# barlettacarmen/CrCNN

Measured on NVIDIA B200. Metric: encrypted MNIST images/sec, higher is better.
Workload: dtype u64

## Files before the change

### crcnn_b200/csrc/engine.cu

```cuda
#include <cuda_runtime.h>
#include <dlfcn.h>
#include <algorithm>
#include <cstdlib>
#include <cstring>
#include <map>
#include <unordered_map>
#include <string>
#include <vector>

#include "../../include/crcnn_b200.h"
#include "kernels.cuh"
#include "params.h"
#include "tc_mac.cuh"
#include "tcn_mac.cuh"
#include "relin32.cuh"
#include "reenc.cuh"

using namespace crcnn;

namespace {

enum KernelClass {
    KC_NTT_FWD = 0, KC_NTT_INV, KC_MAC, KC_PLAIN_EXPAND, KC_POOL, KC_BN, KC_PLAIN_OP,
    KC_BEHZ_LIFT, KC_SQ_TENSOR, KC_BEHZ_FLOOR, KC_RELIN, KC_PROBE, KC_TC_SPLIT, KC_TC_MAC, KC_TCN_SPLIT, KC_TCN_MAC, KC_RELIN32, KC_REENC, KC_COUNT
};
const char *kClassNames[KC_COUNT] = {"ntt_forward", "ntt_inverse", "weighted_sum_mac", "plain_expand_ntt", "pool_sum",
                                     "batch_norm", "plain_op", "behz_lift", "square_tensor", "behz_floor_sk",
                                     "relinearize", "imad_probe", "tc_plane_split", "weighted_sum_tc_i8", "tcn_plane_split",
                                     "weighted_sum_tcn_i8", "relinearize_u32", "reencrypt"};

thread_local std::string g_create_error;

}

struct crcnn_tensor {
    long count;
    int size;
    int ntt;
    uint64_t *d;
};

static long next_plain_serial() { static long s = 0; return ++s; }

struct crcnn_plain {
    long serial = next_plain_serial();
    long count;
    bool sparse_shape = false;
    std::vector<uint32_t> off, idx;
    std::vector<uint64_t> val;
    uint32_t *d_off = nullptr, *d_idx = nullptr;
    uint64_t *d_val = nullptr;
    uint64_t *ntt_mul = nullptr;
    uint64_t *ntt_mul_sh = nullptr;
    uint64_t *ntt_add = nullptr;
    uint64_t *coef_add = nullptr;
    int tap_state = 0;
    int tc_state = 0;
    int8_t *tc_A = nullptr;
    int tc_R = 0, tc_Kpad = 0;
    uint8_t *tcn_W = nullptr;
    int tcn_R = 0;
    uint64_t *fused_C = nullptr, *fused_Csh = nullptr, *fused_D = nullptr;
    long fused_scale = 0, fused_mean = 0;
    int add_mult = 1;
    bool dense_only = false;
    crcnn_plain *folded_w = nullptr, *folded_b = nullptr;
    long folded_key[9] = {0, 0, 0, 0, 0, 0, 0, 0, 0};
};

struct crcnn_evk {
    uint64_t *d = nullptr;
    long key_off[MAXK];
    int digits[MAXK];
    int dbc;
    bool has_r32 = false;
    Relin32 r32;
};

struct crcnn_keys {
    uint64_t *sk = nullptr;
    uint64_t *pk = nullptr;
    ReencConsts c;
};

struct crcnn_ctx {
    int device = 0;
    cudaStream_t stream = nullptr;
    HostParams hp;
    DeviceParams *dP = nullptr;
    std::vector<void *> owned;
    int n = 0, logn = 0, K = 0, S = 0;
    int chunk_terms = 1 << 30;
    size_t weight_cache_bytes = 24ull << 30;
    int sm_count = 148;
    int tc_mode = 1;
    int tc_min_fanin = 256;
    int tc_min_outputs = 32;
    int tap_mode = 1;
    int relin_mode = 1;
    int tcn_mode = 1;
    int tcn_fold = 1;
    size_t tc_scratch_bytes = 12ull << 30;
    std::string err;
    std::map<std::vector<int>, int *> index_cache;
    std::unordered_map<void *, size_t> big_size;
    std::multimap<size_t, void *> big_free;
    size_t big_cached = 0, big_cache_cap = 64ull << 30;
    long long st_big_malloc = 0, st_big_hit = 0, st_big_bypass = 0, st_flush = 0, st_small_malloc = 0;
    uint64_t *stage = nullptr;
    size_t stage_bytes = 0;
    bool prof_on = false;
    long launches[KC_COUNT] = {0};
    double ms[KC_COUNT] = {0};
    double work_bytes[KC_COUNT] = {0};
    double work_ops[KC_COUNT] = {0};
    struct Pending { int cls; cudaEvent_t a, b; };
    std::vector<Pending> pending;
    std::vector<cudaEvent_t> event_pool;
};

namespace {

int fail(crcnn_ctx *ctx, int code, const std::string &msg) {
    if (ctx) ctx->err = msg; else g_create_error = msg;
    return code;
}

#define CU(call)                                                                                       \
    do {                                                                                               \
        cudaError_t e__ = (call);                                                                      \
        if (e__ != cudaSuccess) {                                                                      \
            int code__ = (e__ == cudaErrorMemoryAllocation) ? CRCNN_ERR_OUT_OF_MEMORY : CRCNN_ERR_CUDA; \
            return fail(ctx, code__, std::string(#call) + ": " + cudaGetErrorString(e__));            \
        }                                                                                              \
    } while (0)

#define REQUIRE(cond, msg) \
    do { if (!(cond)) return fail(ctx, CRCNN_ERR_INVALID_ARGUMENT, msg); } while (0)

struct ProfScope {
    crcnn_ctx *c; int cls; cudaEvent_t a = nullptr, b = nullptr;
    ProfScope(crcnn_ctx *ctx, int k, double bytes = 0, double ops = 0) : c(ctx), cls(k) {
        c->launches[cls]++;
        c->work_bytes[cls] += bytes;
        c->work_ops[cls] += ops;
        if (!c->prof_on) return;
        auto get = [&]() { cudaEvent_t e; if (!c->event_pool.empty()) { e = c->event_pool.back(); c->event_pool.pop_back(); } else cudaEventCreate(&e); return e; };
        a = get(); b = get();
        cudaEventRecord(a, c->stream);
    }
    ~ProfScope() {
        if (!a) return;
        cudaEventRecord(b, c->stream);
        c->pending.push_back({cls, a, b});
    }
};

void prof_collect(crcnn_ctx *c) {
    for (auto &p : c->pending) {
        cudaEventSynchronize(p.b);
        float t = 0;
        cudaEventElapsedTime(&t, p.a, p.b);
        c->ms[p.cls] += t;
        c->event_pool.push_back(p.a);
        c->event_pool.push_back(p.b);
    }
    c->pending.clear();
}

inline size_t poly_words(const crcnn_ctx *c) { return (size_t)c->K * c->n; }
inline double lp_bytes(const crcnn_ctx *c, double polys) { return polys * c->n * 8.0; }
inline double lp_bfly(const crcnn_ctx *c, double polys) { return polys * (c->n / 2) * c->logn; }

constexpr size_t kBigBlock = 32ull << 20;
void big_cache_flush(crcnn_ctx *ctx) {
    for (auto &kv : ctx->big_free) { ctx->big_size.erase(kv.second); cudaFreeAsync(kv.second, ctx->stream); }
    ctx->big_free.clear();
    ctx->big_cached = 0;
}
int dev_alloc(crcnn_ctx *ctx, size_t bytes, void **out) {
    *out = nullptr;
    if (bytes == 0) return CRCNN_OK;
    if (bytes >= kBigBlock) {
        auto it = ctx->big_free.find(bytes);
        if (it != ctx->big_free.end()) {
            *out = it->second;
            ctx->big_cached -= bytes;
            ctx->big_free.erase(it);
            ctx->st_big_hit++;
            return CRCNN_OK;
        }
        ctx->st_big_malloc++;
    } else {
        ctx->st_small_malloc++;
    }
    cudaError_t e = cudaMallocAsync(out, bytes, ctx->stream);
    if (e == cudaErrorMemoryAllocation && !ctx->big_free.empty()) {
        cudaGetLastError();
        ctx->st_flush++;
        big_cache_flush(ctx);
        e = cudaMallocAsync(out, bytes, ctx->stream);
    }
    CU(e);
    if (bytes >= kBigBlock) ctx->big_size[*out] = bytes;
    return CRCNN_OK;
}
void dev_free(crcnn_ctx *ctx, void *p) {
    if (!p) return;
    auto it = ctx->big_size.find(p);
    if (it != ctx->big_size.end()) {
        if (ctx->big_cached + it->second <= ctx->big_cache_cap) {
            ctx->big_free.insert({it->second, p});
            ctx->big_cached += it->second;
            return;
        }
        ctx->big_size.erase(it);
        ctx->st_big_bypass++;
    }
    cudaFreeAsync(p, ctx->stream);
}

int new_tensor(crcnn_ctx *ctx, long count, int size, int ntt, crcnn_tensor **out) {
    auto *t = new crcnn_tensor{count, size, ntt, nullptr};
    int rc = dev_alloc(ctx, (size_t)count * size * poly_words(ctx) * 8, (void **)&t->d);
    if (rc) { delete t; return rc; }
    *out = t;
    return CRCNN_OK;
}

int ntt_inplace(crcnn_ctx *ctx, uint64_t *d, long npolys, int slot_base, int slot_count, bool inverse) {
    ProfScope ps(ctx, inverse ? KC_NTT_INV : KC_NTT_FWD, 2 * lp_bytes(ctx, npolys), lp_bfly(ctx, npolys));
    CU(launch_ntt(ctx->dP, ctx->logn, d, npolys, slot_base, slot_count, inverse, ctx->stream));
    return CRCNN_OK;
}

int ensure_domain(crcnn_ctx *ctx, crcnn_tensor *t, int want_ntt) {
    if (t->ntt == want_ntt) return CRCNN_OK;
    int rc = ntt_inplace(ctx, t->d, t->count * t->size * ctx->K, 0, ctx->K, !want_ntt);
    if (rc) return rc;
    t->ntt = want_ntt;
    return CRCNN_OK;
}

enum PlainForm { PF_NTT_MUL, PF_NTT_ADD, PF_COEF_ADD };

int expand_range(crcnn_ctx *ctx, crcnn_plain *p, long first, long count, PlainForm f, uint64_t *dst) {
    ProfScope ps(ctx, KC_PLAIN_EXPAND, lp_bytes(ctx, (double)count * ctx->K), f != PF_COEF_ADD ? lp_bfly(ctx, (double)count * ctx->K) : 0);
    CU(launch_plain_expand(ctx->dP, ctx->logn, ctx->K, p->d_off, p->d_idx, p->d_val, first, count,
                           (f == PF_NTT_MUL ? 0 : 1) | (p->sparse_shape ? 2 : 0), f != PF_COEF_ADD, dst, ctx->stream));
    return CRCNN_OK;
}

int ensure_form(crcnn_ctx *ctx, crcnn_plain *p, PlainForm f) {
// ... 173 lines not shown
    TcnSplitArgs s{};
    s.src = w->ntt_mul; s.index = nullptr; s.dst = w->tcn_W; s.item_polys = 1;
    s.R = R; s.Kpad = Kpad; s.planes = 7; s.ncols = Mall; s.slot0 = 0; s.nslots = ctx->K * ctx->n; s.n = ctx->n; s.K = ctx->K;
    {
        ProfScope ps(ctx, KC_TCN_SPLIT, lp_bytes(ctx, (double)w->count * ctx->K) + (double)tcn_w_bytes(7, Mall, Kpad, ctx->K, ctx->n), 0);
        CU(launch_tcn_split(s, ctx->stream));
    }
    dev_free(ctx, w->ntt_mul); w->ntt_mul = nullptr;
    if (w->ntt_mul_sh) { dev_free(ctx, w->ntt_mul_sh); w->ntt_mul_sh = nullptr; }
    w->tcn_R = R;
    return CRCNN_OK;
}

int run_weighted_sum_tcn(crcnn_ctx *ctx, crcnn_tensor *in, crcnn_plain *w, crcnn_plain *b, const int *d_index, int R,
                         int Npos, int Pimg, int m_first, int M, crcnn_tensor *out) {
    int rc = ensure_domain(ctx, in, 1);
    if (!rc) rc = ensure_form(ctx, b, PF_NTT_ADD);
    if (!rc) rc = ensure_tcn_weights(ctx, w, R);
    if (rc) return rc;
    const size_t pw = poly_words(ctx);
    const int Kpad = tcn_kpad(R), ncols = 2 * Npos, total = ctx->K * ctx->n;
    const size_t per_slot = tcn_x_bytes_per_slot(7, ncols, Kpad);
    long chunk = (long)(ctx->tc_scratch_bytes / per_slot) / 32 * 32;
    chunk = std::max<long>(32, std::min<long>(chunk, total));
    uint8_t *scratch = nullptr;
    rc = dev_alloc(ctx, (size_t)chunk * per_slot, (void **)&scratch);
    if (rc) return rc;
    TcnSplitArgs s{};
    s.src = in->d; s.index = d_index; s.dst = scratch; s.item_polys = 2;
    s.R = R; s.Kpad = Kpad; s.planes = 7; s.ncols = ncols; s.n = ctx->n; s.K = ctx->K;
    TcnMacArgs a{};
    a.W = w->tcn_W; a.X = scratch; a.bias = b->ntt_add + (size_t)m_first * pw; a.out = out->d;
    a.Mall = (int)(w->count / R); a.m_first = m_first; a.M = M;
    a.R = R; a.Kpad = Kpad; a.planes = 7; a.ncols = ncols;
    a.Pimg = Pimg; a.Mtotal = M; a.m0 = 0; a.n = ctx->n; a.K = ctx->K;
    a.variant = ctx->tcn_mode >= 2 ? ctx->tcn_mode - 1 : 0;
    a.use_fold = ctx->tcn_fold;
    for (int j = 0; j < ctx->K; j++) a.fold[j] = tcn_fold_make(ctx->hp.d.tab[j].mod.q);
    for (long s0 = 0; s0 < total && !rc; s0 += chunk) {
        const int ns = (int)std::min<long>(chunk, total - s0);
        s.slot0 = a.slot0 = (int)s0; s.nslots = a.nslots = ns;
        const double xbytes = (double)ns * per_slot;
        cudaError_t e;
        { ProfScope ps(ctx, KC_TCN_SPLIT, (double)ncols * R * ns * 8.0 + xbytes, 0); e = launch_tcn_split(s, ctx->stream); }
        if (e == cudaSuccess) {
            ProfScope ps(ctx, KC_TCN_MAC, xbytes + (double)ns * 7 * M * Kpad + (double)ncols * M * ns * 8.0, (double)ns * ncols * M * R * 49.0);
            e = launch_tcn_mac(ctx->dP, a, ctx->sm_count, ctx->stream);
        }
        if (e != cudaSuccess) rc = fail(ctx, CRCNN_ERR_CUDA, std::string("limb-split tensor-core weighted sum: ") + cudaGetErrorString(e));
    }
    dev_free(ctx, scratch);
    if (!rc) out->ntt = 1;
    return rc;
}

int run_weighted_sum(crcnn_ctx *ctx, crcnn_tensor *in, crcnn_plain *w, crcnn_plain *b, const int *d_index, int R,
                     int Npos, int Pimg, int Mall, int m_first, int M, crcnn_tensor *out) {
    if (ctx->tc_mode && R >= ctx->tc_min_fanin && (ctx->tc_mode == 2 || Mall >= ctx->tc_min_outputs) && w->sparse_shape && tc_mac_available() == cudaSuccess) {
        int rc = ensure_tc_form(ctx, w, R);
        if (rc) return rc;
        if (w->tc_state == 1) return run_weighted_sum_tc(ctx, in, w, b, d_index, R, Npos, Pimg, m_first, M, out);
    }
    if (ctx->tcn_mode && tcn_planes_for(ctx->hp.d) == 7 && R <= TCN_MAX_R && w->count % R == 0 && tc_mac_available() == cudaSuccess &&
        (w->tcn_W || tcn_w_bytes(7, (int)(w->count / R), tcn_kpad(R), ctx->K, ctx->n) <= ctx->weight_cache_bytes))
        return run_weighted_sum_tcn(ctx, in, w, b, d_index, R, Npos, Pimg, m_first, M, out);
    int rc = ensure_domain(ctx, in, 1);
    if (rc) return rc;
    rc = ensure_form(ctx, b, PF_NTT_ADD);
    if (rc) return rc;
    MacArgs a{};
    a.x = in->d; a.in_index = d_index; a.out = out->d;
    a.R = R; a.Npos = Npos; a.Pimg = Pimg; a.Mtotal = M; a.K = ctx->K; a.n = ctx->n;
    a.chunk_terms = ctx->chunk_terms;
    const size_t pw = poly_words(ctx);
    const size_t all_bytes = (size_t)w->count * pw * 8;
    if (w->ntt_mul || all_bytes <= ctx->weight_cache_bytes) {
        rc = ensure_form(ctx, w, PF_NTT_MUL);
        if (rc) return rc;
        a.w = w->ntt_mul + (size_t)m_first * R * pw;
        a.bias = b->ntt_add + (size_t)m_first * pw;
        a.M = M; a.m0 = 0;
        ProfScope ps(ctx, KC_MAC, lp_bytes(ctx, ((double)in->count + (double)M * Npos) * 2 * ctx->K + (double)M * R * ctx->K),
                     (double)M * Npos * R * 2 * ctx->K * ctx->n);
        CU(launch_mac(ctx->dP, a, ctx->stream));
        return CRCNN_OK;
    }
    long rows = (long)std::max<size_t>(1, ctx->weight_cache_bytes / ((size_t)R * pw * 8));
    rows = std::min<long>(rows, M);
    uint64_t *scratch = nullptr;
    rc = dev_alloc(ctx, (size_t)rows * R * pw * 8, (void **)&scratch);
    if (rc) return rc;
    for (long m0 = 0; m0 < M; m0 += rows) {
        long cur = std::min<long>(rows, M - m0);
        rc = expand_range(ctx, w, (long)(m_first + m0) * R, cur * R, PF_NTT_MUL, scratch);
        if (rc) break;
        a.w = scratch; a.bias = b->ntt_add + (size_t)(m_first + m0) * pw;
        a.M = (int)cur; a.m0 = (int)m0;
        ProfScope ps(ctx, KC_MAC, lp_bytes(ctx, ((double)in->count + (double)cur * Npos) * 2 * ctx->K + (double)cur * R * ctx->K),
                     (double)cur * Npos * R * 2 * ctx->K * ctx->n);
        cudaError_t e = launch_mac(ctx->dP, a, ctx->stream);
        if (e != cudaSuccess) { rc = fail(ctx, CRCNN_ERR_CUDA, cudaGetErrorString(e)); break; }
    }
    dev_free(ctx, scratch);
    return rc;
}

int upload_rows(crcnn_ctx *ctx, const uint64_t *host, size_t rows, uint64_t *dst, cudaStream_t s) {
    const size_t n = ctx->n;
    if (rows * n * 8 < (8u << 20)) {
        CU(cudaMemcpy2DAsync(dst, n * 8, host, (n + 1) * 8, n * 8, rows, cudaMemcpyHostToDevice, s));
        return CRCNN_OK;
    }
    uint64_t *stage = nullptr;
    CU(cudaMallocAsync((void **)&stage, rows * (n + 1) * 8, s));
    cudaError_t e = cudaMemcpyAsync(stage, host, rows * (n + 1) * 8, cudaMemcpyHostToDevice, s);
    if (e == cudaSuccess) e = launch_strip_pad(stage, dst, (long)rows, (int)n, s);
    cudaFreeAsync(stage, s);
    if (e != cudaSuccess) return fail(ctx, CRCNN_ERR_CUDA, std::string("upload: ") + cudaGetErrorString(e));
    return CRCNN_OK;
}

}

extern "C" {

const char *crcnn_last_error(const crcnn_ctx *ctx) { return ctx ? ctx->err.c_str() : g_create_error.c_str(); }

int crcnn_ctx_create(int n, int K, const uint64_t *q, uint64_t t, int device, crcnn_ctx **out) {
    crcnn_ctx *ctx = nullptr;
    if (!out || !q) return fail(nullptr, CRCNN_ERR_INVALID_ARGUMENT, "null argument");
    *out = nullptr;
    int ndev = 0;
    if (cudaGetDeviceCount(&ndev) != cudaSuccess || ndev == 0)
        return fail(nullptr, CRCNN_ERR_NO_DEVICE, "no CUDA device: crcnn_b200 has no CPU fallback");
    if (device < 0 || device >= ndev) return fail(nullptr, CRCNN_ERR_INVALID_ARGUMENT, "bad device ordinal");
    HostParams hp;
    try {
        hp = derive_params(n, K, q, t);
    } catch (const std::exception &e) {
        return fail(nullptr, CRCNN_ERR_INVALID_ARGUMENT, e.what());
    }
    CU(cudaSetDevice(device));
    auto *c = new crcnn_ctx();
    c->device = device; c->n = n; c->K = K; c->S = hp.d.S; c->logn = hp.d.logn;
    int maxbits = 0;
    for (int i = 0; i < K; i++) { int b = 0; for (uint64_t v = q[i]; v; v >>= 1) b++; maxbits = std::max(maxbits, b); }
    int spare = 128 - 2 * maxbits;
    c->chunk_terms = spare >= 30 ? (1 << 30) : (1 << spare);
    cudaDeviceGetAttribute(&c->sm_count, cudaDevAttrMultiProcessorCount, device);
    if (const char *e = getenv("CRCNN_TC")) c->tc_mode = atoi(e);
    if (const char *e = getenv("CRCNN_TCN")) c->tcn_mode = atoi(e);
    if (const char *e = getenv("CRCNN_TAP")) c->tap_mode = atoi(e);
    if (const char *e = getenv("CRCNN_TCN_FOLD")) c->tcn_fold = atoi(e);
    cudaMemPool_t pool;
    if (cudaDeviceGetDefaultMemPool(&pool, device) == cudaSuccess) {
        uint64_t thr = UINT64_MAX;
        cudaMemPoolSetAttribute(pool, cudaMemPoolAttrReleaseThreshold, &thr);
    }
    {
        size_t fr = 0, tot = 0;
        if (cudaMemGetInfo(&fr, &tot) == cudaSuccess && tot) c->big_cache_cap = tot / 4 * 3;
    }
    int slots = K + hp.d.S;
    auto up = [&](const std::vector<uint64_t> &v, const uint64_t **dst) -> cudaError_t {
        void *d = nullptr;
        cudaError_t e = cudaMalloc(&d, v.size() * 8);
        if (e != cudaSuccess) return e;
        c->owned.push_back(d);
        *dst = (const uint64_t *)d;
        return cudaMemcpy(d, v.data(), v.size() * 8, cudaMemcpyHostToDevice);
    };
    cudaError_t e = cudaSuccess;
    for (int s = 0; s < slots && e == cudaSuccess; s++) {
        std::vector<uint64_t> fw(2 * (size_t)n), bw(2 * (size_t)n);
        for (int i = 0; i < n; i++) {
            fw[2 * i] = hp.w[s][i]; fw[2 * i + 1] = hp.wp[s][i];
            bw[2 * i] = hp.iwf[s][i]; bw[2 * i + 1] = hp.iwfp[s][i];
        }
        e = up(fw, &hp.d.tab[s].w);
        if (e == cudaSuccess) e = up(bw, &hp.d.tab[s].iw);
        const int NG = n >> 4;
        std::vector<uint64_t> fl(2 * (size_t)16 * NG, 0), bl(2 * (size_t)16 * NG, 0);
        for (int G = 0; G < NG; G++)
            for (int st = 0; st < 4; st++) {
                for (int lb = 0; lb < (1 << st); lb++) {
                    const size_t at = 2 * ((size_t)((1 << st) - 1 + lb) * NG + G), from = 2 * ((((size_t)NG + G) << st) + lb);
                    fl[at] = fw[from]; fl[at + 1] = fw[from + 1];
                }
                for (int lb = 0; lb < (1 << (3 - st)); lb++) {
                    const size_t at = 2 * ((size_t)(16 - (16 >> st) + lb) * NG + G);
                    const size_t from = 2 * ((size_t)((n >> 1) >> st) + ((size_t)G << (3 - st)) + lb);
                    bl[at] = bw[from]; bl[at + 1] = bw[from + 1];
                }
            }
        if (e == cudaSuccess) e = up(fl, &hp.d.tab[s].wl);
        if (e == cudaSuccess) e = up(bl, &hp.d.tab[s].iwl);
        hp.d.tab[s].tf = nullptr;
        if (e == cudaSuccess && s < K) e = up(hp.tf[s], &hp.d.tab[s].tf);
    }
    if (e == cudaSuccess) e = cudaMalloc((void **)&c->dP, sizeof(DeviceParams));
    if (e == cudaSuccess) e = cudaMemcpy(c->dP, &hp.d, sizeof(DeviceParams), cudaMemcpyHostToDevice);
    if (e != cudaSuccess) {
        std::string m = cudaGetErrorString(e);
        for (void *p : c->owned) cudaFree(p);
        if (c->dP) cudaFree(c->dP);
        delete c;
        return fail(nullptr, CRCNN_ERR_CUDA, "context setup: " + m);
    }
    c->hp = std::move(hp);
    *out = c;
    return CRCNN_OK;
}

int crcnn_ctx_destroy(crcnn_ctx *ctx) {
    if (!ctx) return CRCNN_OK;
    cudaSetDevice(ctx->device);
    big_cache_flush(ctx);
    cudaStreamSynchronize(ctx->stream);
    prof_collect(ctx);
    for (auto e : ctx->event_pool) cudaEventDestroy(e);
    for (auto &kv : ctx->index_cache) cudaFree(kv.second);
    if (ctx->stage) cudaFree(ctx->stage);
    for (void *p : ctx->owned) cudaFree(p);
    cudaFree(ctx->dP);
    delete ctx;
    return CRCNN_OK;
}

int crcnn_ctx_set_stream(crcnn_ctx *ctx, void *cuda_stream) {
    if (!ctx) return CRCNN_ERR_INVALID_ARGUMENT;
    CU(cudaStreamSynchronize(ctx->stream));
    ctx->stream = (cudaStream_t)cuda_stream;
    return CRCNN_OK;
}

int crcnn_ctx_sync(crcnn_ctx *ctx) {
    if (!ctx) return CRCNN_ERR_INVALID_ARGUMENT;
    CU(cudaStreamSynchronize(ctx->stream));
    prof_collect(ctx);
    return CRCNN_OK;
}

int crcnn_ctx_alloc_stats(crcnn_ctx *ctx, long long out[6]) {
    if (!ctx || !out) return CRCNN_ERR_INVALID_ARGUMENT;
    out[0] = ctx->st_big_malloc; out[1] = ctx->st_big_hit; out[2] = ctx->st_big_bypass; out[3] = ctx->st_flush;
    out[4] = ctx->st_small_malloc; out[5] = (long long)ctx->big_cached;
    return CRCNN_OK;
}

int crcnn_ctx_set_weight_cache_bytes(crcnn_ctx *ctx, size_t bytes) {
    if (!ctx) return CRCNN_ERR_INVALID_ARGUMENT;
    ctx->weight_cache_bytes = bytes;
    return CRCNN_OK;
}

int crcnn_ctx_set_tensor_core_mode(crcnn_ctx *ctx, int mode, int min_fanin, size_t scratch_bytes) {
    if (!ctx) return CRCNN_ERR_INVALID_ARGUMENT;
    REQUIRE(mode >= 0 && mode <= 2, "tensor-core mode must be 0, 1 or 2");
    ctx->tc_mode = mode;
    if (min_fanin > 0) ctx->tc_min_fanin = min_fanin;
    if (scratch_bytes > 0) ctx->tc_scratch_bytes = scratch_bytes;
    return CRCNN_OK;
}

int crcnn_ctx_set_limb_split_mode(crcnn_ctx *ctx, int mode) {
    if (!ctx) return CRCNN_ERR_INVALID_ARGUMENT;
    REQUIRE(mode >= 0 && mode <= 3, "limb-split mode must be 0 (off), 1 (on), 2 (row-major kernel) or 3 (column-major kernel)");
    ctx->tcn_mode = mode;
    return CRCNN_OK;
}

int crcnn_ctx_set_limb_split_reduction(crcnn_ctx *ctx, int mode) {
    if (!ctx) return CRCNN_ERR_INVALID_ARGUMENT;
    REQUIRE(mode == 0 || mode == 1, "limb-split reduction must be 0 (128-bit recombination + Barrett) or 1 (folded through 2^k - delta)");
    ctx->tcn_fold = mode;
    return CRCNN_OK;
}

int crcnn_ctx_set_relin_mode(crcnn_ctx *ctx, int mode) {
    if (!ctx) return CRCNN_ERR_INVALID_ARGUMENT;
    REQUIRE(mode == 0 || mode == 1, "relinearize mode must be 0 (64-bit transforms) or 1 (word-size auxiliary primes)");
    ctx->relin_mode = mode;
    return CRCNN_OK;
}

int crcnn_ctx_ntt_table(const crcnn_ctx *ctx_c, int slot, int which, uint64_t *out) {
    crcnn_ctx *ctx = const_cast<crcnn_ctx *>(ctx_c);
    if (!ctx) return CRCNN_ERR_INVALID_ARGUMENT;
    REQUIRE(out && slot >= 0 && slot < ctx->K + ctx->S && which >= 0 && which < 4, "bad table selector");
    const auto &v = which == 0 ? ctx->hp.w[slot] : which == 1 ? ctx->hp.wp[slot] : which == 2 ? ctx->hp.iw[slot] : ctx->hp.iwp[slot];
    memcpy(out, v.data(), v.size() * 8);
    return CRCNN_OK;
}

int crcnn_ctx_bsk_count(const crcnn_ctx *ctx) { return ctx ? ctx->S : CRCNN_ERR_INVALID_ARGUMENT; }

int crcnn_tensor_upload_ex(crcnn_ctx *ctx, const uint64_t *host, long count, int size, int ntt_form, crcnn_tensor **out) {
    if (!ctx) return CRCNN_ERR_INVALID_ARGUMENT;
    REQUIRE(host && out && count >= 0 && size >= 2 && size <= 3, "bad tensor upload arguments");
    CU(cudaSetDevice(ctx->device));
    crcnn_tensor *t = nullptr;
    int rc = new_tensor(ctx, count, size, ntt_form ? 1 : 0, &t);
    if (rc) return rc;
    const size_t n = ctx->n, rows = (size_t)count * size * ctx->K;
    if (rows) {
        int rc2 = upload_rows(ctx, host, rows, t->d, ctx->stream);
// ... 602 lines not shown
    rc = new_tensor(ctx, Nout, 2, 1, &o);
    if (rc) return rc;
    {
        ProfScope ps(ctx, KC_POOL, lp_bytes(ctx, ((double)in->count + Nout) * 2 * ctx->K), (double)Nout * (R + 1) * 2 * ctx->K * ctx->n);
        cudaError_t e = launch_pool(ctx->dP, ctx->n, ctx->K, in->d, d_index, Nout, R, invstd->fused_C, invstd->fused_Csh, true, o->d, ctx->stream,
                                    xo * yo, zd, invstd->fused_D);
        if (e != cudaSuccess) { crcnn_tensor_free(ctx, o); return fail(ctx, CRCNN_ERR_CUDA, cudaGetErrorString(e)); }
    }
    *out = o;
    return CRCNN_OK;
}

int crcnn_conv_pool_bn_forward_shard(crcnn_ctx *ctx, crcnn_tensor *in, crcnn_plain *w, crcnn_plain *b, int batch, int xd, int yd, int zd,
                                     int xs, int ys, int xf, int yf, int nf, int pxs, int pys, int pxf, int pyf, crcnn_plain *scale,
                                     crcnn_plain *mean, crcnn_plain *invstd, int k0, int kc, crcnn_tensor **out) {
    if (!ctx) return CRCNN_ERR_INVALID_ARGUMENT;
    REQUIRE(k0 >= 0 && kc >= 0 && k0 + kc <= nf, "bad output-channel shard");
    REQUIRE(in && w && b && mean && invstd && out, "null argument");
    REQUIRE(batch > 0 && xd > 0 && yd > 0 && zd > 0 && xs > 0 && ys > 0 && xf > 0 && yf > 0 && nf > 0 && xf <= xd && yf <= yd,
            "bad convolution geometry");
    const int cxo = (xd - xf) / xs + 1, cyo = (yd - yf) / ys + 1;
    REQUIRE(pxs > 0 && pys > 0 && pxf > 0 && pyf > 0 && pxf <= cxo && pyf <= cyo, "bad pooling geometry");
    const int pxo = (cxo - pxf) / pxs + 1, pyo = (cyo - pyf) / pys + 1;
    const int Rp = pxf * pyf, R = zd * xf * yf;
    REQUIRE(in->size == 2 && in->count == (long)batch * zd * xd * yd, "input tensor does not match the layer geometry");
    REQUIRE(w->count == (long)nf * R && b->count == nf, "kernel/bias count does not match the layer geometry");
    REQUIRE((!scale || scale->count >= 1) && mean->count == nf && invstd->count == nf, "mean/var count does not match the channel count");
    CU(cudaSetDevice(ctx->device));
    const bool pooled_grid = pxs <= pxf && pys <= pyf && xs <= xf && ys <= yf && pxs * xs <= xf && pys * ys <= yf && Rp <= 64 && sum_fits_64(ctx, Rp) &&
                             ctx->tcn_mode && tcn_planes_for(ctx->hp.d) == 7 && R <= TCN_MAX_R && tc_mac_available() == cudaSuccess &&
                             tcn_w_bytes(7, nf, tcn_kpad(R), ctx->K, ctx->n) <= ctx->weight_cache_bytes && !getenv("CRCNN_NO_POOLED_CONV");
    if (!pooled_grid) {
        if (k0 != 0 || kc != nf)
            return fail(ctx, CRCNN_ERR_UNSUPPORTED, "channel shards of conv + pool + batch-norm need the pooled-grid path");
        crcnn_tensor *mid = nullptr;
        int rc = crcnn_conv_forward(ctx, in, w, b, batch, xd, yd, zd, xs, ys, xf, yf, nf, &mid);
        if (rc) return rc;
        rc = crcnn_pool_bn_forward(ctx, mid, batch, cxo, cyo, nf, pxs, pys, pxf, pyf, scale, mean, invstd, out);
        crcnn_tensor_free(ctx, mid);
        return rc;
    }
    int rc = ensure_pool_bn_consts(ctx, scale, mean, invstd);
    if (rc) return rc;
    const long key[9] = {b->serial, scale ? scale->serial : -1, mean->serial, invstd->serial, (long)Rp, 0, 0, 0, 0};
    if (!w->folded_w || memcmp(key, w->folded_key, sizeof(key)) != 0) {
        if (w->folded_w) { crcnn_plain_free(ctx, w->folded_w); w->folded_w = nullptr; }
        if (w->folded_b) { crcnn_plain_free(ctx, w->folded_b); w->folded_b = nullptr; }
        const size_t pw = poly_words(ctx);
        rc = make_plain(ctx, std::vector<uint32_t>(w->off), std::vector<uint32_t>(w->idx), std::vector<uint64_t>(w->val), &w->folded_w);
        if (rc) return rc;
        w->folded_w->sparse_shape = false;
        w->folded_w->tc_state = -1; w->folded_w->tap_state = -1;
        rc = ensure_form(ctx, w->folded_w, PF_NTT_MUL);
        if (rc) return rc;
        CU(launch_fold_affine(ctx->dP, w->folded_w->ntt_mul, (long)nf * R, (long)pw, R, invstd->fused_C, nullptr, ctx->stream));
        rc = ensure_tcn_weights(ctx, w->folded_w, R);
        if (rc) return rc;
        rc = make_plain(ctx, std::vector<uint32_t>(b->off), std::vector<uint32_t>(b->idx), std::vector<uint64_t>(b->val), &w->folded_b);
        if (rc) return rc;
        w->folded_b->add_mult = Rp;
        rc = ensure_form(ctx, w->folded_b, PF_NTT_ADD);
        if (rc) return rc;
        CU(launch_fold_affine(ctx->dP, w->folded_b->ntt_add, (long)nf, (long)pw, 1, invstd->fused_C, invstd->fused_D, ctx->stream));
        memcpy(w->folded_key, key, sizeof(key));
    }
    const int sxd = xd - (pxf - 1) * xs, syd = yd - (pyf - 1) * ys;
    const int Nsum = batch * zd * sxd * syd;
    std::vector<int> skey = {4, batch, xd, yd, zd, xs, ys, pxf, pyf};
    const int *d_index = nullptr;
    if (ctx->index_cache.find(skey) == ctx->index_cache.end()) {
        std::vector<int> table((size_t)Nsum * Rp);
        size_t o = 0;
        for (int bz = 0; bz < batch * zd; bz++)
            for (int u = 0; u < sxd; u++)
                for (int v = 0; v < syd; v++)
                    for (int a = 0; a < pxf; a++)
                        for (int c = 0; c < pyf; c++) table[o++] = (bz * xd + u + a * xs) * yd + v + c * ys;
        rc = get_index_table(ctx, skey, table, &d_index);
        if (rc) return rc;
    } else {
        d_index = ctx->index_cache[skey];
    }
    crcnn_tensor *sums = nullptr, *pooled = nullptr;
    rc = new_tensor(ctx, Nsum, 2, in->ntt, &sums);
    if (rc) return rc;
    {
        ProfScope ps(ctx, KC_POOL, lp_bytes(ctx, ((double)in->count + Nsum) * 2 * ctx->K), (double)Nsum * Rp * 2 * ctx->K * ctx->n);
        cudaError_t e = launch_pool(ctx->dP, ctx->n, ctx->K, in->d, d_index, Nsum, Rp, nullptr, nullptr, true, sums->d, ctx->stream);
        if (e != cudaSuccess) { crcnn_tensor_free(ctx, sums); return fail(ctx, CRCNN_ERR_CUDA, cudaGetErrorString(e)); }
    }
    rc = crcnn_conv_forward_shard(ctx, sums, w->folded_w, w->folded_b, batch, sxd, syd, zd, pxs * xs, pys * ys, xf, yf, nf, k0, kc, &pooled);
    crcnn_tensor_free(ctx, sums);
    if (rc) return rc;
    if (pooled->count != (long)batch * kc * pxo * pyo || !pooled->ntt) {
        crcnn_tensor_free(ctx, pooled);
        return fail(ctx, CRCNN_ERR_UNSUPPORTED, "pooled-grid convolution produced an unexpected shape");
    }
    *out = pooled;
    return CRCNN_OK;
}

int crcnn_conv_pool_bn_forward(crcnn_ctx *ctx, crcnn_tensor *in, crcnn_plain *w, crcnn_plain *b, int batch, int xd, int yd, int zd,
                               int xs, int ys, int xf, int yf, int nf, int pxs, int pys, int pxf, int pyf, crcnn_plain *scale,
                               crcnn_plain *mean, crcnn_plain *invstd, crcnn_tensor **out) {
    return crcnn_conv_pool_bn_forward_shard(ctx, in, w, b, batch, xd, yd, zd, xs, ys, xf, yf, nf, pxs, pys, pxf, pyf, scale, mean, invstd, 0, nf, out);
}

int crcnn_bn_forward(crcnn_ctx *ctx, crcnn_tensor *in, int batch, int zd, int xd, int yd, crcnn_plain *mean,
                     crcnn_plain *invstd, crcnn_tensor **out) {
    if (!ctx) return CRCNN_ERR_INVALID_ARGUMENT;
    REQUIRE(in && mean && invstd && out, "null argument");
    REQUIRE(batch > 0 && zd > 0 && xd > 0 && yd > 0, "bad batch-norm geometry");
    REQUIRE(in->size == 2 && in->count == (long)batch * zd * xd * yd, "input tensor does not match the layer geometry");
    REQUIRE(mean->count == zd && invstd->count == zd, "mean/var count does not match the channel count");
    CU(cudaSetDevice(ctx->device));
    if (!in->ntt && ctx->tap_mode && tap_eligible(ctx, invstd)) {
        int rc = ensure_form(ctx, mean, PF_COEF_ADD);
        if (rc) return rc;
        crcnn_tensor *o = nullptr;
        rc = new_tensor(ctx, in->count, 2, 0, &o);
        if (rc) return rc;
        TapMulArgs a{};
        a.in = in->d; a.in_index = nullptr; a.R = 1; a.sub = mean->coef_add;
        a.t_off = invstd->d_off; a.t_idx = invstd->d_idx; a.t_val = invstd->d_val; a.per_channel = xd * yd; a.channels = zd;
        a.out = o->d; a.nout = in->count;
        ProfScope ps(ctx, KC_BN, lp_bytes(ctx, (double)in->count * 4 * ctx->K), (double)in->count * 2 * ctx->K * ctx->n);
        cudaError_t e = launch_tapmul(ctx->dP, ctx->n, ctx->K, a, ctx->stream);
        if (e != cudaSuccess) { crcnn_tensor_free(ctx, o); return fail(ctx, CRCNN_ERR_CUDA, cudaGetErrorString(e)); }
        *out = o;
        return CRCNN_OK;
    }
    int rc = ensure_domain(ctx, in, 1);
    if (!rc) rc = ensure_form(ctx, mean, PF_NTT_ADD);
    if (!rc) rc = ensure_shoup(ctx, invstd);
    if (rc) return rc;
    crcnn_tensor *o = nullptr;
    rc = new_tensor(ctx, in->count, 2, 1, &o);
    if (rc) return rc;
    {
        ProfScope ps(ctx, KC_BN, lp_bytes(ctx, (double)in->count * 4 * ctx->K), (double)in->count * 2 * ctx->K * ctx->n);
        cudaError_t e = launch_bn(ctx->dP, ctx->n, ctx->K, in->d, in->count, xd * yd, zd, mean->ntt_add, invstd->ntt_mul, invstd->ntt_mul_sh, o->d, ctx->stream);
        if (e != cudaSuccess) { crcnn_tensor_free(ctx, o); return fail(ctx, CRCNN_ERR_CUDA, cudaGetErrorString(e)); }
    }
    *out = o;
    return CRCNN_OK;
}

int crcnn_square(crcnn_ctx *ctx, crcnn_tensor *in, crcnn_tensor **out3) {
    if (!ctx) return CRCNN_ERR_INVALID_ARGUMENT;
    REQUIRE(in && out3, "null argument");
    REQUIRE(in->size == 2, "square expects size-2 ciphertexts");
    CU(cudaSetDevice(ctx->device));
    const bool have_ntt = in->ntt != 0;
    crcnn_tensor *o = nullptr;
    int rc = new_tensor(ctx, in->count, 3, 0, &o);
    if (rc) return rc;
    const int KS = ctx->K + ctx->S;
    const size_t n = ctx->n, pw = poly_words(ctx);
    const long step = std::max<long>(1, std::min<long>(in->count, (long)((2ull << 30) / (5 * (size_t)KS * n * 8))));
    uint64_t *ext = nullptr, *prod = nullptr, *coef = nullptr;
    rc = dev_alloc(ctx, (size_t)step * 2 * KS * n * 8, (void **)&ext);
    if (!rc) rc = dev_alloc(ctx, (size_t)step * 3 * KS * n * 8, (void **)&prod);
    if (!rc && have_ntt) rc = dev_alloc(ctx, (size_t)step * 2 * pw * 8, (void **)&coef);
    if (rc) { crcnn_tensor_free(ctx, o); return rc; }
    for (long c0 = 0; c0 < in->count && !rc; c0 += step) {
        const long cur = std::min<long>(step, in->count - c0);
        const uint64_t *src = in->d + c0 * 2 * pw;
        cudaError_t e = cudaSuccess;
        if (have_ntt) {
            ProfScope ps(ctx, KC_NTT_INV, 2 * lp_bytes(ctx, (double)cur * 2 * ctx->K), lp_bfly(ctx, (double)cur * 2 * ctx->K));
            e = launch_ntt_grouped(ctx->dP, ctx->logn, coef, cur * 2 * ctx->K, 0, ctx->K, true, ctx->K, 0, ctx->stream, src);
        }
        if (e == cudaSuccess) { ProfScope ps(ctx, KC_BEHZ_LIFT, lp_bytes(ctx, (double)cur * 2 * (ctx->K + (have_ntt ? ctx->S : KS))), (double)cur * 2 * n * ctx->S * (ctx->K + 1)); e = launch_behz_lift(ctx->hp.d, ctx->n, have_ntt ? coef : src, have_ntt ? src : nullptr, cur, ext, ctx->stream); }
        if (e == cudaSuccess) {
            if (have_ntt) {
                ProfScope ps(ctx, KC_NTT_FWD, 2 * lp_bytes(ctx, (double)cur * 2 * ctx->S), lp_bfly(ctx, (double)cur * 2 * ctx->S));
                e = launch_ntt_grouped(ctx->dP, ctx->logn, ext, cur * 2 * ctx->S, ctx->K, ctx->S, false, KS, ctx->K, ctx->stream);
            } else {
                ProfScope ps(ctx, KC_NTT_FWD, 2 * lp_bytes(ctx, (double)cur * 2 * KS), lp_bfly(ctx, (double)cur * 2 * KS));
                e = launch_ntt(ctx->dP, ctx->logn, ext, cur * 2 * KS, 0, KS, false, ctx->stream);
            }
        }
        if (e == cudaSuccess) {
            ProfScope ps(ctx, KC_SQ_TENSOR, lp_bytes(ctx, (double)cur * 5 * KS), lp_bfly(ctx, (double)cur * 3 * KS));
            e = launch_ntt_inv_tensor(ctx->dP, ctx->logn, ext, have_ntt ? src : nullptr, cur, KS, prod, ctx->stream);
        }
        if (e == cudaSuccess) { ProfScope ps(ctx, KC_BEHZ_FLOOR, lp_bytes(ctx, (double)cur * 3 * (KS + ctx->K)),
                                                     (double)cur * 3 * n * (ctx->S * (ctx->K + 1) + ctx->S + ctx->K * ctx->S)); e = launch_behz_floor(ctx->hp.d, ctx->n, prod, cur, o->d + c0 * 3 * pw, ctx->stream); }
        if (e != cudaSuccess) rc = fail(ctx, CRCNN_ERR_CUDA, cudaGetErrorString(e));
    }
    dev_free(ctx, coef);
    dev_free(ctx, ext); dev_free(ctx, prod);
    if (rc) { crcnn_tensor_free(ctx, o); return rc; }
    *out3 = o;
    return CRCNN_OK;
}

int crcnn_relinearize(crcnn_ctx *ctx, crcnn_tensor *in3, crcnn_evk *evk, crcnn_tensor **out2) {
    if (!ctx) return CRCNN_ERR_INVALID_ARGUMENT;
    REQUIRE(in3 && evk && out2, "null argument");
    REQUIRE(in3->size == 3, "relinearize expects size-3 ciphertexts");
    int total_digits = 0;
    for (int i = 0; i < ctx->K; i++) {
        int bits = 0; for (uint64_t v = ctx->hp.d.tab[i].mod.q; v; v >>= 1) bits++;
        REQUIRE(evk->digits[i] * evk->dbc >= bits, "not enough evaluation keys");
        total_digits += evk->digits[i];
    }
    REQUIRE(total_digits <= 63, "too many key digits for 128-bit lazy accumulation");
    CU(cudaSetDevice(ctx->device));
    int rc = ensure_domain(ctx, in3, 0);
    if (rc) return rc;
    crcnn_tensor *o = nullptr;
    rc = new_tensor(ctx, in3->count, 2, 0, &o);
    if (rc) return rc;
    const size_t pw = poly_words(ctx);
    if (evk->has_r32 && ctx->relin_mode == 1) {
        const Relin32Consts &c = evk->r32.c;
        const size_t per_ct = relin32_scratch_bytes(ctx->n, ctx->K, c);
        const long step = std::max<long>(1, std::min<long>(std::min<long>(in3->count, 200000), (long)((2ull << 30) / per_ct)));
        void *scratch = nullptr;
        rc = dev_alloc(ctx, (size_t)step * per_ct, &scratch);
        if (rc) { crcnn_tensor_free(ctx, o); return rc; }
        for (long c0 = 0; c0 < in3->count && !rc; c0 += step) {
            const long cnt = std::min<long>(step, in3->count - c0);
            ProfScope ps(ctx, KC_RELIN32, lp_bytes(ctx, (double)cnt * 5 * ctx->K),
                         lp_bfly(ctx, (double)cnt * (c.D + 2 * ctx->K) * c.S3));
            cudaError_t e = relin32_run(ctx->dP, ctx->logn, ctx->K, evk->r32, in3->d + c0 * 3 * pw, o->d + c0 * 2 * pw, cnt, scratch, ctx->stream);
            if (e != cudaSuccess) rc = fail(ctx, CRCNN_ERR_CUDA, cudaGetErrorString(e));
        }
        dev_free(ctx, scratch);
        if (rc) { crcnn_tensor_free(ctx, o); return rc; }
        *out2 = o;
        return CRCNN_OK;
    }
    RelinArgs a{};
    a.evk = evk->d; a.dbc = evk->dbc;
    for (int i = 0; i < MAXK; i++) { a.key_off[i] = evk->key_off[i]; a.digits[i] = evk->digits[i]; }
    const size_t per_ct = (size_t)(1 + total_digits + 2) * pw * 8;
    const long step = std::max<long>(1, std::min<long>(in3->count, (long)((2ull << 30) / per_ct)));
    uint64_t *scratch = nullptr;
    rc = dev_alloc(ctx, (size_t)step * per_ct, (void **)&scratch);
    if (rc) { crcnn_tensor_free(ctx, o); return rc; }
    a.dsc = scratch;
    a.dig = scratch + (size_t)step * pw;
    a.acc = a.dig + (size_t)step * total_digits * pw;
    for (long c0 = 0; c0 < in3->count && !rc; c0 += step) {
        a.count = std::min<long>(step, in3->count - c0);
        a.in3 = in3->d + c0 * 3 * pw;
        a.out = o->d + c0 * 2 * pw;
        cudaError_t e;
        { ProfScope ps(ctx, KC_RELIN, lp_bytes(ctx, (double)a.count * 3 * ctx->K), lp_bfly(ctx, (double)a.count * total_digits * ctx->K)); e = launch_relin(ctx->dP, ctx->logn, ctx->K, a, ctx->stream); }
        if (e == cudaSuccess) {
            ProfScope ps(ctx, KC_NTT_INV, 2 * lp_bytes(ctx, (double)a.count * 2 * ctx->K) + lp_bytes(ctx, (double)a.count * 2 * ctx->K), lp_bfly(ctx, (double)a.count * 2 * ctx->K));
            e = launch_ntt_grouped(ctx->dP, ctx->logn, a.out, a.count * 2 * ctx->K, 0, ctx->K, true, ctx->K, 0, ctx->stream, a.acc, a.in3,
                                   2 * ctx->K, 3 * ctx->K);
        }
        if (e != cudaSuccess) rc = fail(ctx, CRCNN_ERR_CUDA, cudaGetErrorString(e));
    }
    dev_free(ctx, scratch);
    if (rc) { crcnn_tensor_free(ctx, o); return rc; }
    *out2 = o;
    return CRCNN_OK;
}

int crcnn_square_forward(crcnn_ctx *ctx, crcnn_tensor *in, crcnn_evk *evk, crcnn_tensor **out) {
    if (!ctx) return CRCNN_ERR_INVALID_ARGUMENT;
    crcnn_tensor *t3 = nullptr;
    int rc = crcnn_square(ctx, in, &t3);
    if (rc) return rc;
    rc = crcnn_relinearize(ctx, t3, evk, out);
    crcnn_tensor_free(ctx, t3);
    return rc;
}

int crcnn_transform_to_ntt(crcnn_ctx *ctx, crcnn_tensor *t) {
    if (!ctx) return CRCNN_ERR_INVALID_ARGUMENT;
    REQUIRE(t, "null argument");
    REQUIRE(!t->ntt, "tensor is already in NTT form");
    CU(cudaSetDevice(ctx->device));
    return ensure_domain(ctx, t, 1);
}
int crcnn_transform_from_ntt(crcnn_ctx *ctx, crcnn_tensor *t) {
    if (!ctx) return CRCNN_ERR_INVALID_ARGUMENT;
    REQUIRE(t, "null argument");
    REQUIRE(t->ntt, "tensor is not in NTT form");
    CU(cudaSetDevice(ctx->device));
    return ensure_domain(ctx, t, 0);
}

int crcnn_plain_op(crcnn_ctx *ctx, crcnn_tensor *t, crcnn_plain *p, long index, int op) {
    if (!ctx) return CRCNN_ERR_INVALID_ARGUMENT;
    REQUIRE(t && p && index >= 0 && index < p->count && op >= 0 && op <= 2, "bad plain_op arguments");
    CU(cudaSetDevice(ctx->device));
    int rc;
    const uint64_t *pl, *pl_sh = nullptr;
    if (op == 0) {
        rc = ensure_domain(ctx, t, 1);
        if (!rc) rc = ensure_shoup(ctx, p);
        if (rc) return rc;
        pl = p->ntt_mul + index * poly_words(ctx);
        pl_sh = p->ntt_mul_sh + index * poly_words(ctx);
    } else {
        rc = ensure_form(ctx, p, t->ntt ? PF_NTT_ADD : PF_COEF_ADD);
        if (rc) return rc;
        pl = (t->ntt ? p->ntt_add : p->coef_add) + index * poly_words(ctx);
    }
    ProfScope ps(ctx, KC_PLAIN_OP, lp_bytes(ctx, (double)t->count * (op == 0 ? t->size : 1) * 2 * ctx->K), (double)t->count * (op == 0 ? t->size : 1) * ctx->K * ctx->n);
    CU(launch_plain_op(ctx->dP, ctx->n, ctx->K, t->d, t->count, t->size, pl, pl_sh, op, ctx->stream));
    return CRCNN_OK;
}

int crcnn_add_many(crcnn_ctx *ctx, crcnn_tensor *t, crcnn_tensor **out) {
    if (!ctx) return CRCNN_ERR_INVALID_ARGUMENT;
    REQUIRE(t && out, "null argument");
    REQUIRE(t->count >= 1, "encrypteds cannot be empty");
    REQUIRE(t->size == 2, "add_many is implemented for size-2 ciphertexts");
    CU(cudaSetDevice(ctx->device));
    auto pass = [&](const uint64_t *src, long first, int nout, int g, uint64_t *dst) -> int {
        std::vector<int> key = {4, (int)first, nout, g};
        const int *d_index = nullptr;
        auto it = ctx->index_cache.find(key);
        if (it == ctx->index_cache.end()) {
            std::vector<int> table((size_t)nout * g);
            for (size_t i = 0; i < table.size(); i++) table[i] = (int)(first + (long)i);
            int rc = get_index_table(ctx, key, table, &d_index);
            if (rc) return rc;
        } else d_index = it->second;
        ProfScope ps(ctx, KC_POOL, lp_bytes(ctx, ((double)nout * g + nout) * 2 * ctx->K), (double)nout * g * 2 * ctx->K * ctx->n);
        CU(launch_pool(ctx->dP, ctx->n, ctx->K, src, d_index, nout, g, nullptr, nullptr, sum_fits_64(ctx, g), dst, ctx->stream));
        return CRCNN_OK;
    };
    crcnn_tensor *o = nullptr;
    int rc = new_tensor(ctx, 1, 2, t->ntt, &o);
    if (rc) return rc;
    if (t->count <= 128) {
        rc = pass(t->d, 0, 1, (int)t->count, o->d);
    } else {
        int g = 1;
        while ((long)g * g < t->count) g++;
        const long full = t->count / g, tail = t->count % g, groups = full + (tail ? 1 : 0);
        crcnn_tensor *part = nullptr;
// ... 395 lines not shown
```

### crcnn_b200/csrc/host_selftest.cpp

```cpp
#include <cinttypes>
#include <cstdio>
#include <cstdlib>
#include <vector>
#include "params.h"

using namespace crcnn;

static uint64_t fnv(const std::vector<uint64_t> &v) {
    uint64_t h = 1469598103934665603ULL;
    for (uint64_t x : v) { h ^= x; h *= 1099511628211ULL; }
    return h;
}

int main(int argc, char **argv) {
    if (argc < 4) { fprintf(stderr, "usage: host_selftest n t q...\n"); return 2; }
    int n = atoi(argv[1]);
    uint64_t t = strtoull(argv[2], nullptr, 0);
    std::vector<uint64_t> q;
    for (int i = 3; i < argc; i++) q.push_back(strtoull(argv[i], nullptr, 0));
    try {
        HostParams hp = derive_params(n, (int)q.size(), q.data(), t);
        const DeviceParams &d = hp.d;
        printf("K %d L %d S %d half %" PRIu64 "\n", d.K, d.L, d.S, d.half);
        for (int s = 0; s < d.K + d.S; s++) {
            printf("slot %d q %" PRIu64 " r0 %" PRIu64 " r1 %" PRIu64 " root %" PRIu64 " w %" PRIu64 " wp %" PRIu64 " iw %" PRIu64 " iwp %" PRIu64 "\n",
                   s, d.tab[s].mod.q, d.tab[s].mod.r0, d.tab[s].mod.r1, hp.roots[s], fnv(hp.w[s]), fnv(hp.wp[s]), fnv(hp.iw[s]), fnv(hp.iwp[s]));
        }
        for (int j = 0; j < d.K; j++)
            printf("prime %d delta %" PRIu64 " rho %" PRIu64 " lift %" PRIu64 "\n", j, d.delta[j], d.rho[j], d.lift_inc[j]);
        uint64_t x = 0x123456789abcdef1ULL, y = 0xfedcba9876543211ULL;
        for (int s = 0; s < d.K + d.S; s++) {
            const Mod &m = d.tab[s].mod;
            for (int it = 0; it < 1000; it++) {
                x = x * 6364136223846793005ULL + 1442695040888963407ULL;
                y = y * 2862933555777941757ULL + 3037000493ULL;
                uint64_t a = x % (4 * m.q), b = y % m.q;
                uint64_t want = (uint64_t)(((unsigned __int128)a * b) % m.q);
                if (mulmod(a, b, m) != want) { printf("MULMOD MISMATCH\n"); return 1; }
                uint64_t wp = (uint64_t)((((unsigned __int128)b) << 64) / m.q);
                uint64_t lazy = mulshoup_lazy(a, b, wp, m.q);
                if (lazy >= 2 * m.q || lazy % m.q != want) { printf("SHOUP MISMATCH\n"); return 1; }
            }
        }
        for (int j = 0; j < d.K; j++) {
            const Mod &m = d.tab[j].mod;
            const TcnFold f = tcn_fold_make(m.q);
            printf("fold %d ok %u T %u delta %u\n", j, f.ok, f.T, f.delta);
            if (!f.ok) continue;
            for (int it = 0; it < 200000; it++) {
                uint32_t s[13];
                const int mode = it % 8;
                for (int w = 0; w < 13; w++) {
                    x = x * 6364136223846793005ULL + 1442695040888963407ULL;
                    const uint32_t r = (uint32_t)(x >> 33);
                    s[w] = mode == 0 ? 0x7fffffffu : mode == 1 ? 0u : mode == 2 ? ((x >> 20) & 1 ? 0x7fffffffu : 0u)
                         : mode == 3 ? 7u * 4096u * 255u * 255u - (r & 3) : mode == 4 ? (r >> (x & 31)) : r;
                }
                y = y * 2862933555777941757ULL + 3037000493ULL;
                const uint64_t bias = mode == 0 ? m.q - 1 : (it & 1) ? y % m.q : 0;
                unsigned __int128 z = 0;
                for (int w = 12; w >= 0; w--) z = (z << 8) + s[w];
                const uint64_t want = (uint64_t)((z + bias) % m.q);
                if (tcn_fold_reduce(s, bias, f, m.q) != want) { printf("FOLD MISMATCH\n"); return 1; }
            }
        }
        for (int sidx = 0; sidx < d.K + d.S; sidx++) {
            const Mod &m = d.tab[sidx].mod;
            const Fold128 f = fold128_make(m.q);
            printf("fold128 %d ok %u delta %u\n", sidx, f.ok, f.delta);
            if (!f.ok) continue;
            for (int it = 0; it < 200000; it++) {
                x = x * 6364136223846793005ULL + 1442695040888963407ULL;
                y = y * 2862933555777941757ULL + 3037000493ULL;
                U128 z;
                const int mode = it % 8;
                z.lo = mode == 0 ? ~0ull : mode == 1 ? 0 : mode == 2 ? m.q - 1 : mode == 3 ? m.q : x;
                z.hi = mode == 0 ? ~0ull : mode == 1 ? 0 : mode == 2 ? 0 : mode == 3 ? (y >> (y & 63)) : mode == 4 ? (y >> 40) : y;
                const uint64_t want = (uint64_t)(((((unsigned __int128)z.hi) << 64) | z.lo) % m.q);
                if (reduce128_fold(z, f) != want || barrett128(z, m) != want) { printf("FOLD128 MISMATCH\n"); return 1; }
            }
        }
        for (int i = 4; i >= 0; i--) {
            double vals[] = {0.0867, -3.25, 0.0, 1.0, 2.8215};
            std::vector<uint32_t> idx; std::vector<uint64_t> val;
            encode_fractional_sparse(vals[i], n, t, idx, val);
            printf("enc %.4f nnz %zu", vals[i], idx.size());
            for (size_t e = 0; e < idx.size(); e++) printf(" %u:%" PRIu64, idx[e], val[e]);
            printf("\n");
        }
        printf("OK\n");
    } catch (const std::exception &e) {
        printf("ERROR %s\n", e.what());
        return 1;
    }
    return 0;
}
```

### crcnn_b200/csrc/kernels.cu

```cuda
#include "kernels.cuh"
#include "devcfg.cuh"
#include "ntt.cuh"
#include <cstdlib>

namespace crcnn {

template <int LOGN>
__global__ void __launch_bounds__(NttPlan<LOGN>::THREADS, NttPlan<LOGN>::MIN_CTAS)
ntt_fwd_kernel(uint64_t *__restrict__ data, const DeviceParams *__restrict__ P, int slot_base, int slot_count, int group_polys,
               int group_off) {
    extern __shared__ uint64_t sm[];
    const long p = blockIdx.x;
    const NttTable tb = P->tab[slot_base + (int)(p % slot_count)];
    uint64_t *poly = data + ((p / slot_count) * group_polys + group_off + p % slot_count) * (1L << LOGN);
    ntt_forward_to_smem<LOGN>(sm, poly, tb);
    smem_store_poly_canonical<LOGN>(sm, poly, tb.mod);
}

template <int LOGN>
__global__ void __launch_bounds__(NttPlan<LOGN>::THREADS, NttPlan<LOGN>::MIN_CTAS)
ntt_inv_kernel(uint64_t *__restrict__ data, const DeviceParams *__restrict__ P, int slot_base, int slot_count, int group_polys,
               int group_off, const uint64_t *__restrict__ src, const uint64_t *__restrict__ addend, int add_group, int add_stride) {
    extern __shared__ uint64_t sm[];
    const long p = blockIdx.x;
    const NttTable tb = P->tab[slot_base + (int)(p % slot_count)];
    const long off = ((p / slot_count) * group_polys + group_off + p % slot_count) * (1L << LOGN);
    uint64_t *poly = data + off;
    smem_load_poly<LOGN>(sm, src ? src + off : poly);
    __syncthreads();
    ntt_inverse_from_smem<LOGN>(sm, poly, tb, addend ? addend + ((p / add_group) * add_stride + p % add_group) * (1L << LOGN) : nullptr);
}

template <int LOGN>
__global__ void __launch_bounds__(NttPlan<LOGN>::THREADS, NttPlan<LOGN>::MIN_CTAS)
ntt_inv_tensor_kernel(const DeviceParams *__restrict__ P, const uint64_t *__restrict__ ext, const uint64_t *__restrict__ qntt, int KS,
                      uint64_t *__restrict__ prod) {
    extern __shared__ uint64_t sm[];
    constexpr int N = 1 << LOGN;
    const long b = blockIdx.x;
    const int j = (int)(b % KS);
    const int k = (int)((b / KS) % 3);
    const long ct = b / (3L * KS);
    const NttTable tb = P->tab[j];
    const uint64_t *c0 = ext + ((ct * 2) * KS + j) * N, *c1 = c0 + (long)KS * N;
    if (qntt && j < P->K) {
        c0 = qntt + ((ct * 2) * P->K + j) * N;
        c1 = c0 + (long)P->K * N;
    }
    if (k == 1) {
#pragma unroll 8
        for (int i = threadIdx.x; i < N; i += NttPlan<LOGN>::THREADS) {
            const uint64_t ab = mulmod(__ldg(c0 + i), __ldg(c1 + i), tb.mod);
            sm[ntt_pad(i)] = addmod(ab, ab, tb.mod.q);
        }
    } else {
        const uint64_t *c = k == 0 ? c0 : c1;
#pragma unroll 8
        for (int i = threadIdx.x; i < N; i += NttPlan<LOGN>::THREADS) {
            const uint64_t a = __ldg(c + i);
            sm[ntt_pad(i)] = mulmod(a, a, tb.mod);
        }
    }
    __syncthreads();
    ntt_inverse_from_smem<LOGN>(sm, prod + b * N, tb);
}

template <int LOGN>
static cudaError_t launch_ntt_inv_tensor_t(const DeviceParams *P, const uint64_t *ext, const uint64_t *qntt, long count, int KS, uint64_t *prod,
                                           cudaStream_t stream) {
    using Pl = NttPlan<LOGN>;
    const size_t smem = Pl::SMEM_WORDS * sizeof(uint64_t);
    auto kf = ntt_inv_tensor_kernel<LOGN>;
    static DeviceOnce once;
    if (once.first()) {
        cudaFuncSetAttribute(kf, cudaFuncAttributeMaxDynamicSharedMemorySize, (int)smem);
        cudaFuncSetAttribute(kf, cudaFuncAttributePreferredSharedMemoryCarveout, cudaSharedmemCarveoutMaxShared);
    }
    kf<<<(unsigned)(count * 3 * KS), Pl::THREADS, smem, stream>>>(P, ext, qntt, KS, prod);
    return cudaGetLastError();
}

cudaError_t launch_ntt_inv_tensor(const DeviceParams *P, int logn, const uint64_t *ext, const uint64_t *qntt, long count, int KS, uint64_t *prod,
                                  cudaStream_t stream) {
    if (count <= 0) return cudaSuccess;
    switch (logn) {
        case 10: return launch_ntt_inv_tensor_t<10>(P, ext, qntt, count, KS, prod, stream);
        case 11: return launch_ntt_inv_tensor_t<11>(P, ext, qntt, count, KS, prod, stream);
        case 12: return launch_ntt_inv_tensor_t<12>(P, ext, qntt, count, KS, prod, stream);
        case 13: return launch_ntt_inv_tensor_t<13>(P, ext, qntt, count, KS, prod, stream);
        case 14: return launch_ntt_inv_tensor_t<14>(P, ext, qntt, count, KS, prod, stream);
        default: return cudaErrorInvalidValue;
    }
}

template <int LOGN>
static cudaError_t launch_ntt_t(const DeviceParams *P, uint64_t *data, long npolys, int slot_base, int slot_count,
                                bool inverse, int group_polys, int group_off, const uint64_t *src, const uint64_t *addend,
                                int add_group, int add_stride, cudaStream_t stream) {
    using Pl = NttPlan<LOGN>;
    size_t smem = Pl::SMEM_WORDS * sizeof(uint64_t);
    auto kf = ntt_fwd_kernel<LOGN>;
    auto ki = ntt_inv_kernel<LOGN>;
    static DeviceOnce once;
    if (once.first()) {
        cudaFuncSetAttribute(kf, cudaFuncAttributeMaxDynamicSharedMemorySize, (int)smem);
        cudaFuncSetAttribute(ki, cudaFuncAttributeMaxDynamicSharedMemorySize, (int)smem);
        cudaFuncSetAttribute(kf, cudaFuncAttributePreferredSharedMemoryCarveout, cudaSharedmemCarveoutMaxShared);
        cudaFuncSetAttribute(ki, cudaFuncAttributePreferredSharedMemoryCarveout, cudaSharedmemCarveoutMaxShared);
    }
    if (npolys <= 0) return cudaSuccess;
    if ((src || addend) && !inverse) return cudaErrorInvalidValue;
    if (inverse) ki<<<(unsigned)npolys, Pl::THREADS, smem, stream>>>(data, P, slot_base, slot_count, group_polys, group_off, src, addend, add_group, add_stride);
    else kf<<<(unsigned)npolys, Pl::THREADS, smem, stream>>>(data, P, slot_base, slot_count, group_polys, group_off);
    return cudaGetLastError();
}

cudaError_t launch_ntt_grouped(const DeviceParams *P, int logn, uint64_t *data, long npolys, int slot_base, int slot_count,
                               bool inverse, int group_polys, int group_off, cudaStream_t stream, const uint64_t *src,
                               const uint64_t *addend, int add_group, int add_stride) {
    switch (logn) {
        case 10: return launch_ntt_t<10>(P, data, npolys, slot_base, slot_count, inverse, group_polys, group_off, src, addend, add_group, add_stride, stream);
        case 11: return launch_ntt_t<11>(P, data, npolys, slot_base, slot_count, inverse, group_polys, group_off, src, addend, add_group, add_stride, stream);
        case 12: return launch_ntt_t<12>(P, data, npolys, slot_base, slot_count, inverse, group_polys, group_off, src, addend, add_group, add_stride, stream);
        case 13: return launch_ntt_t<13>(P, data, npolys, slot_base, slot_count, inverse, group_polys, group_off, src, addend, add_group, add_stride, stream);
        case 14: return launch_ntt_t<14>(P, data, npolys, slot_base, slot_count, inverse, group_polys, group_off, src, addend, add_group, add_stride, stream);
        default: return cudaErrorInvalidValue;
    }
}

cudaError_t launch_ntt(const DeviceParams *P, int logn, uint64_t *data, long npolys, int slot_base, int slot_count,
                       bool inverse, cudaStream_t stream) {
    return launch_ntt_grouped(P, logn, data, npolys, slot_base, slot_count, inverse, slot_count, 0, stream);
}

template <int LOGN>
__global__ void __launch_bounds__(NttPlan<LOGN>::THREADS, NttPlan<LOGN>::MIN_CTAS)
plain_expand_kernel(const DeviceParams *__restrict__ P, int K, const uint32_t *__restrict__ offsets,
                    const uint32_t *__restrict__ idx, const uint64_t *__restrict__ val, long first, int mode,
                    int to_ntt, uint64_t *__restrict__ out) {
    extern __shared__ uint64_t sm[];
    constexpr int N = 1 << LOGN;
    const long b = blockIdx.x;
    const long pi = b / K;
    const int j = (int)(b % K);
    const NttTable tb = P->tab[j];
    const uint64_t half = P->half;
    const int sparse_shape = (mode >> 1) & 1;
    mode &= 1;
    for (int i = threadIdx.x; i < NttPlan<LOGN>::SMEM_WORDS; i += blockDim.x) sm[i] = 0;
    __syncthreads();
    const uint32_t lo = offsets[first + pi], hi = offsets[first + pi + 1];
    auto residue = [&](uint64_t c) -> uint64_t {
        if (mode == 0) return c >= half ? c + P->lift_inc[j] : c;
        U128 z = mul128(P->delta[j], c);
        if (c >= half) add128_64(z, P->rho[j]);
        return barrett128(z, tb.mod);
    };
    uint64_t *dst = out + b * N;
    if (to_ntt && sparse_shape) {
        constexpr int SKIP = sparse_skip_stages(LOGN);
        constexpr int NB = 1 << SKIP, M = N >> SKIP;
        const uint32_t cnt = (hi - lo) * NB;
        for (uint32_t w = threadIdx.x; w < cnt; w += blockDim.x) {
            const uint32_t e = lo + w / NB, blk = w % NB;
            const int ix = (int)idx[e];
            uint64_t v = residue(val[e]);
            if (ix < 64) {
                sm[ntt_pad((int)blk * M + ix)] = v;
            } else {
                sm[ntt_pad((int)blk * M + M - (N - ix))] = mulmod(v, __ldg(tb.tf + blk), tb.mod);
            }
        }
        __syncthreads();
        ntt_forward_in_smem<LOGN, NttPlan<LOGN>::skip_passes()>(sm, tb);
        smem_store_poly_canonical<LOGN>(sm, dst, tb.mod);
        return;
    }
    for (uint32_t e = lo + threadIdx.x; e < hi; e += blockDim.x) sm[ntt_pad((int)idx[e])] = residue(val[e]);
    __syncthreads();
    if (to_ntt) {
        ntt_forward_in_smem<LOGN>(sm, tb);
        smem_store_poly_canonical<LOGN>(sm, dst, tb.mod);
    } else {
        for (int i = threadIdx.x; i < N; i += blockDim.x) dst[i] = sm[ntt_pad(i)];
    }
}

template <int LOGN>
static cudaError_t launch_plain_expand_t(const DeviceParams *P, int K, const uint32_t *offsets, const uint32_t *idx,
                                         const uint64_t *val, long first, long count, int mode, bool to_ntt,
                                         uint64_t *out, cudaStream_t stream) {
    using Pl = NttPlan<LOGN>;
    size_t smem = Pl::SMEM_WORDS * sizeof(uint64_t);
    auto k = plain_expand_kernel<LOGN>;
    static DeviceOnce once;
    if (once.first()) {
        cudaFuncSetAttribute(k, cudaFuncAttributeMaxDynamicSharedMemorySize, (int)smem);
        cudaFuncSetAttribute(k, cudaFuncAttributePreferredSharedMemoryCarveout, cudaSharedmemCarveoutMaxShared);
    }
    if (count <= 0) return cudaSuccess;
    k<<<(unsigned)(count * K), Pl::THREADS, smem, stream>>>(P, K, offsets, idx, val, first, mode, to_ntt ? 1 : 0, out);
    return cudaGetLastError();
}

cudaError_t launch_plain_expand(const DeviceParams *P, int logn, int K, const uint32_t *offsets, const uint32_t *idx,
                                const uint64_t *val, long first, long count, int mode, bool to_ntt, uint64_t *out,
                                cudaStream_t stream) {
    switch (logn) {
        case 10: return launch_plain_expand_t<10>(P, K, offsets, idx, val, first, count, mode, to_ntt, out, stream);
        case 11: return launch_plain_expand_t<11>(P, K, offsets, idx, val, first, count, mode, to_ntt, out, stream);
        case 12: return launch_plain_expand_t<12>(P, K, offsets, idx, val, first, count, mode, to_ntt, out, stream);
        case 13: return launch_plain_expand_t<13>(P, K, offsets, idx, val, first, count, mode, to_ntt, out, stream);
        case 14: return launch_plain_expand_t<14>(P, K, offsets, idx, val, first, count, mode, to_ntt, out, stream);
        default: return cudaErrorInvalidValue;
    }
}

constexpr int MAC_THREADS = 128;

template <int TM, int TN>
__global__ void __launch_bounds__(MAC_THREADS, (TM * TN <= 4) ? 4 : 2)
mac_kernel(const DeviceParams *__restrict__ P, MacArgs a) {
    extern __shared__ int s_idx[];
    const int n = a.n, K = a.K, R = a.R;
    const int slices_per_limb = n / MAC_THREADS;
    const int j = blockIdx.y / slices_per_limb;
    const int c = (blockIdx.y % slices_per_limb) * MAC_THREADS + threadIdx.x;
    const int tiles_m = (a.M + TM - 1) / TM;
    const int tiles_n = (a.Npos + TN - 1) / TN;
    const int tn = blockIdx.x % tiles_n, tm = blockIdx.x / tiles_n;
    (void)tiles_m;
    const int m_base = tm * TM, p_base = tn * TN;
    const Mod mod = P->tab[j].mod;
    const long limb_off = (long)j * n + c;
    const long poly_words = (long)K * n;

    for (int i = threadIdx.x; i < TN * R; i += MAC_THREADS) {
        int t = i / R, r = i - t * R;
        int p = min(p_base + t, a.Npos - 1);
        s_idx[i] = a.in_index[(long)p * R + r];
    }
    __syncthreads();

    Acc7 acc[TM][TN][2];
#pragma unroll
    for (int m = 0; m < TM; m++)
#pragma unroll
        for (int t = 0; t < TN; t++) { acc[m][t][0] = acc7_zero(); acc[m][t][1] = acc7_zero(); }

    const unsigned w_step = (unsigned)(poly_words * 8), ct_step = (unsigned)(2 * poly_words * 8);
    const char *wptr[TM];
#pragma unroll
    for (int m = 0; m < TM; m++)
        wptr[m] = reinterpret_cast<const char *>(a.w + (long)min(m_base + m, a.M - 1) * R * poly_words + limb_off);
    const char *x0 = reinterpret_cast<const char *>(a.x + limb_off);
    const char *x1 = x0 + w_step;

    for (int r0 = 0; r0 < R; r0 += a.chunk_terms) {
        const int r1 = min(R, r0 + a.chunk_terms);
#pragma unroll 2
        for (int r = r0; r < r1; r++) {
            uint64_t W[TM], X[TN][2];
#pragma unroll
            for (int m = 0; m < TM; m++) { W[m] = __ldg(reinterpret_cast<const uint64_t *>(wptr[m])); wptr[m] += w_step; }
#pragma unroll
            for (int t = 0; t < TN; t++) {
                const unsigned long long off = (unsigned long long)(unsigned)s_idx[t * R + r] * ct_step;
                X[t][0] = __ldg(reinterpret_cast<const uint64_t *>(x0 + off));
                X[t][1] = __ldg(reinterpret_cast<const uint64_t *>(x1 + off));
            }
#pragma unroll
            for (int m = 0; m < TM; m++)
#pragma unroll
                for (int t = 0; t < TN; t++) {
                    mac7(acc[m][t][0], X[t][0], W[m]);
                    mac7(acc[m][t][1], X[t][1], W[m]);
                }
        }
// ... 262 lines not shown
                    if (R == 4) { v.x += w[u][1].x + w[u][2].x + w[u][3].x; v.y += w[u][1].y + w[u][2].y + w[u][3].y; }
                    finish(i2, v, R > 1);
                }
            }
        }
    } else {
        for (int i2 = threadIdx.x; i2 < PAIRS; i2 += 256) {
            const int cc = wrap_cc(i2);
            ulonglong2 v = make_ulonglong2(0, 0);
            for (int r = 0; r < R; r++) {
                const uint64_t *src = R <= 16 ? s_src[r] + cc
                                              : a.in + (long)__ldg(a.in_index + o * a.R + r) * ctw + (long)poly * pw + (long)j * n + cc;
                const ulonglong2 x2 = __ldg(reinterpret_cast<const ulonglong2 *>(src));
                v.x += x2.x; v.y += x2.y;
            }
            finish(i2, v, true);
        }
    }
    __syncthreads();
    const int npos = t_count[0], nneg = t_count[1];
    const uint64_t *base = sm + 64 + threadIdx.x;
    uint64_t pos[4] = {0, 0, 0, 0}, neg[4] = {0, 0, 0, 0};
    for (int e = 0; e < npos; e++) {
        const uint64_t *v = base + t_delta[e];
#pragma unroll
        for (int k = 0; k < 4; k++) pos[k] += v[256 * k];
    }
    for (int e = npos; e < npos + nneg; e++) {
        const uint64_t *v = base + t_delta[e];
#pragma unroll
        for (int k = 0; k < 4; k++) neg[k] += v[256 * k];
    }
    const uint64_t off = (uint64_t)nneg * mod.q;
    uint64_t *op = a.out + o * ctw + (long)poly * pw + (long)j * n + c0 + threadIdx.x;
#pragma unroll
    for (int k = 0; k < 4; k++) op[256 * k] = reduce64(pos[k] + off - neg[k], mod);
}

cudaError_t launch_tapmul(const DeviceParams *P, int n, int K, const TapMulArgs &a, cudaStream_t stream) {
    if (a.nout <= 0) return cudaSuccess;
    const long blocks = a.nout * 2 * K * (n / TAP_CT);
    if (n % TAP_CT || blocks > 0x7fffffffL) return cudaErrorInvalidValue;
    tapmul_kernel<<<(unsigned)blocks, 256, 0, stream>>>(P, a);
    return cudaGetLastError();
}

__global__ void __launch_bounds__(256)
shoup_companion_kernel(const DeviceParams *__restrict__ P, const uint64_t *__restrict__ data, long words, uint64_t *__restrict__ out) {
    const long w = (long)blockIdx.x * 256 + threadIdx.x;
    if (w >= words) return;
    const uint64_t q = P->tab[(w / P->n) % P->K].mod.q;
    out[w] = (uint64_t)((((unsigned __int128)__ldg(data + w)) << 64) / q);
}

cudaError_t launch_shoup_companion(const DeviceParams *P, const uint64_t *data, long words, uint64_t *out, cudaStream_t stream) {
    if (words <= 0) return cudaSuccess;
    shoup_companion_kernel<<<(unsigned)((words + 255) / 256), 256, 0, stream>>>(P, data, words, out);
    return cudaGetLastError();
}

__global__ void __launch_bounds__(256)
scale_small_kernel(const DeviceParams *__restrict__ P, uint64_t *__restrict__ data, long words, int times) {
    const long w = (long)blockIdx.x * 256 + threadIdx.x;
    if (w >= words) return;
    const uint64_t q = P->tab[(w / P->n) % P->K].mod.q;
    const uint64_t v = data[w];
    uint64_t acc = 0;
    for (int i = 0; i < times; i++) acc = addmod(acc, v, q);
    data[w] = acc;
}

__global__ void __launch_bounds__(256)
fold_affine_kernel(const DeviceParams *__restrict__ P, uint64_t *__restrict__ data, long rows, int group, const uint64_t *__restrict__ C,
                   const uint64_t *__restrict__ D) {
    const long pw = (long)P->K * P->n;
    const long w = (long)blockIdx.x * 256 + threadIdx.x;
    if (w >= rows * pw) return;
    const long row = w / pw, lw = w - row * pw;
    const Mod mod = P->tab[lw / P->n].mod;
    const long cw = (row / group) * pw + lw;
    uint64_t v = mulmod(data[w], __ldg(C + cw), mod);
    if (D) v = submod(v, __ldg(D + cw), mod.q);
    data[w] = v;
}

cudaError_t launch_fold_affine(const DeviceParams *P, uint64_t *data, long rows, long poly_words, int group, const uint64_t *C,
                               const uint64_t *D, cudaStream_t stream) {
    if (rows <= 0) return cudaSuccess;
    fold_affine_kernel<<<(unsigned)((rows * poly_words + 255) / 256), 256, 0, stream>>>(P, data, rows, group, C, D);
    return cudaGetLastError();
}

__global__ void __launch_bounds__(256)
fold_fc_input_affine_kernel(const DeviceParams *__restrict__ P, uint64_t *__restrict__ W, int out_dim, int in_dim, int per_channel,
                            const uint64_t *__restrict__ C, const uint64_t *__restrict__ D, uint64_t *__restrict__ Bias) {
    const long pw = (long)P->K * P->n;
    const long id = (long)blockIdx.x * 256 + threadIdx.x;
    if (id >= (long)out_dim * pw) return;
    const long k = id / pw, lw = id - k * pw;
    const Mod mod = P->tab[lw / P->n].mod;
    uint64_t acc = Bias[k * pw + lw];
    for (int r = 0; r < in_dim; r++) {
        const long cw = (long)(r / per_channel) * pw + lw;
        uint64_t *wp = W + ((long)k * in_dim + r) * pw + lw;
        const uint64_t w = *wp;
        acc = submod(acc, mulmod(w, __ldg(D + cw), mod), mod.q);
        *wp = mulmod(w, __ldg(C + cw), mod);
    }
    Bias[k * pw + lw] = acc;
}

cudaError_t launch_fold_fc_input_affine(const DeviceParams *P, uint64_t *W, int out_dim, int in_dim, long poly_words, int per_channel,
                                        const uint64_t *C, const uint64_t *D, uint64_t *Bias, cudaStream_t stream) {
    if (out_dim <= 0 || in_dim <= 0) return cudaSuccess;
    fold_fc_input_affine_kernel<<<(unsigned)((out_dim * poly_words + 255) / 256), 256, 0, stream>>>(P, W, out_dim, in_dim, per_channel, C, D, Bias);
    return cudaGetLastError();
}

cudaError_t launch_scale_small(const DeviceParams *P, uint64_t *data, long words, int times, cudaStream_t stream) {
    if (words <= 0) return cudaSuccess;
    scale_small_kernel<<<(unsigned)((words + 255) / 256), 256, 0, stream>>>(P, data, words, times);
    return cudaGetLastError();
}

__global__ void __launch_bounds__(256)
plain_op_kernel(const DeviceParams *__restrict__ P, uint64_t *__restrict__ data, int size, const uint64_t *__restrict__ pl,
                const uint64_t *__restrict__ pl_sh, int op) {
    const int n = P->n, K = P->K;
    const long pw = (long)K * n, ctw = size * pw, active = op == 0 ? ctw : pw;
    const long ct = blockIdx.x;
    const long word = ((long)blockIdx.y * 256 + threadIdx.x) * 4;
    if (word >= active) return;
    const long lw = word % pw;
    const int j = (int)(lw / n);
    const Mod mod = P->tab[j].mod;
    ulonglong2 *x = reinterpret_cast<ulonglong2 *>(data + ct * ctw + word);
    const ulonglong2 *w = reinterpret_cast<const ulonglong2 *>(pl + lw);
    ulonglong2 a = x[0], b = x[1];
    const ulonglong2 wa = __ldg(w), wb = __ldg(w + 1);
    if (op == 0) {
        const ulonglong2 *ws = reinterpret_cast<const ulonglong2 *>(pl_sh + lw);
        const ulonglong2 sa = __ldg(ws), sb = __ldg(ws + 1);
        uint64_t r;
        r = mulshoup_lazy(a.x, wa.x, sa.x, mod.q); a.x = r >= mod.q ? r - mod.q : r;
        r = mulshoup_lazy(a.y, wa.y, sa.y, mod.q); a.y = r >= mod.q ? r - mod.q : r;
        r = mulshoup_lazy(b.x, wb.x, sb.x, mod.q); b.x = r >= mod.q ? r - mod.q : r;
        r = mulshoup_lazy(b.y, wb.y, sb.y, mod.q); b.y = r >= mod.q ? r - mod.q : r;
    }
    else if (op == 1) { a.x = addmod(a.x, wa.x, mod.q); a.y = addmod(a.y, wa.y, mod.q); b.x = addmod(b.x, wb.x, mod.q); b.y = addmod(b.y, wb.y, mod.q); }
    else { a.x = submod(a.x, wa.x, mod.q); a.y = submod(a.y, wa.y, mod.q); b.x = submod(b.x, wb.x, mod.q); b.y = submod(b.y, wb.y, mod.q); }
    x[0] = a; x[1] = b;
}

template <bool FOLD>
__device__ __forceinline__ uint64_t behz_reduce(U128 z, const Mod &m) {
    if constexpr (FOLD) {
        Fold128 f;
        const int k = 64 - __clzll((long long)m.q);
        f.q = m.q; f.delta = (uint32_t)((1ull << k) - m.q); f.sh = (uint32_t)(k - 32); f.mask = (1u << (k - 32)) - 1; f.ok = 1;
        return reduce128_fold(z, f);
    } else {
        return barrett128(z, m);
    }
}
template <bool FOLD>
__device__ __forceinline__ uint64_t behz_mulmod(uint64_t a, uint64_t b, const Mod &m) { return behz_reduce<FOLD>(mul128(a, b), m); }

template <int KT, int ST, bool FOLD>
__global__ void __launch_bounds__(128)
behz_lift_kernel(const __grid_constant__ DeviceParams P, const uint64_t *__restrict__ in, const uint64_t *__restrict__ in_ntt,
                 uint64_t *__restrict__ ext) {
    const int n = P.n, K = KT ? KT : P.K, S = KT ? ST : P.S;
    constexpr int KB = KT ? KT : MAXK, SB = KT ? ST : MAXS;
    const int per = n / 128;
    const long poly = blockIdx.x / per;
    const int c = (blockIdx.x % per) * 128 + threadIdx.x;
    const uint64_t *src = in + poly * K * n + c;
    uint64_t *dst = ext + poly * (K + S) * n + c;
    uint64_t y[KB];
    uint32_t zmt = 0;
#pragma unroll
    for (int i = 0; i < KB; i++) {
        if (i < K) {
            uint64_t x = __ldg(src + (long)i * n);
            if (!in_ntt) dst[(long)i * n] = x;
            y[i] = behz_mulmod<FOLD>(x, P.mt_inv_qhat[i], P.tab[i].mod);
            zmt += (uint32_t)y[i] * (uint32_t)P.qhat_mod_mt[i];
        }
    }
    const uint32_t r = zmt * (uint32_t)P.neg_inv_q_mod_mt;
#pragma unroll
    for (int k = 0; k < SB; k++) {
        if (k < S) {
            Acc7 acc = acc7_zero();
#pragma unroll
            for (int i = 0; i < KB; i++)
                if (i < K) mac7(acc, y[i], P.lift_a[k][i]);
            mac7(acc, (uint64_t)r, P.lift_b[k]);
            dst[(long)(K + k) * n] = behz_reduce<FOLD>(acc7_value(acc), P.tab[K + k].mod);
        }
    }
}

template <int KT, int ST, bool FOLD>
__global__ void __launch_bounds__(128)
behz_floor_kernel(const __grid_constant__ DeviceParams P, const uint64_t *__restrict__ prod, uint64_t *__restrict__ out) {
    const int n = P.n, K = KT ? KT : P.K, S = KT ? ST : P.S, L = S - 1;
    constexpr int KB = KT ? KT : MAXK, SB = KT ? ST : MAXS;
    const int per = n / 128;
    const long poly = blockIdx.x / per;
    const int c = (blockIdx.x % per) * 128 + threadIdx.x;
    const uint64_t *src = prod + poly * (K + S) * n + c;
    uint64_t *dst = out + poly * K * n + c;
    uint64_t u[KB], g[SB];
#pragma unroll
    for (int i = 0; i < KB; i++)
        if (i < K) u[i] = behz_mulmod<FOLD>(__ldg(src + (long)i * n), P.fl_c[i], P.tab[i].mod);
    uint64_t f_sk = 0;
#pragma unroll
    for (int k = 0; k < SB; k++)
        if (k < S) {
            Acc7 acc = acc7_zero();
            mac7(acc, __ldg(src + (long)(K + k) * n), P.fl_T[k]);
#pragma unroll
            for (int i = 0; i < KB; i++)
                if (i < K) mac7(acc, u[i], P.fl_N[k][i]);
            uint64_t v = behz_reduce<FOLD>(acc7_value(acc), P.tab[K + k].mod);
            if (k < L) g[k] = v; else f_sk = v;
        }
    const Mod msk = P.tab[K + L].mod;
    Acc7 acc = acc7_zero();
#pragma unroll
    for (int i = 0; i < SB; i++)
        if (i < L) mac7(acc, g[i], P.fl_P[i]);
    mac7(acc, msk.q - f_sk, P.inv_M_mod_msk);
    const uint64_t alpha = behz_reduce<FOLD>(acc7_value(acc), msk);
    const bool centered_neg = alpha > (msk.q >> 1);
    const uint64_t alpha_mag = centered_neg ? msk.q - alpha : alpha;
#pragma unroll
    for (int j = 0; j < KB; j++)
        if (j < K) {
            Acc7 e = acc7_zero();
#pragma unroll
            for (int i = 0; i < SB; i++)
                if (i < L) mac7(e, g[i], P.Mhat_mod_q[j][i]);
            mac7(e, alpha_mag, centered_neg ? P.M_mod_q[j] : P.neg_M_mod_q[j]);
            dst[(long)j * n] = behz_reduce<FOLD>(acc7_value(e), P.tab[j].mod);
        }
}

__global__ void __launch_bounds__(256)
relin_scale_kernel(const DeviceParams *__restrict__ P, const uint64_t *__restrict__ in3, uint64_t *__restrict__ dsc) {
    const int n = P->n, K = P->K;
    const long pw = (long)K * n;
    const long ct = blockIdx.x;
    const long lw = (long)blockIdx.y * 256 + threadIdx.x;
    const int i = (int)(lw / n);
    dsc[ct * pw + lw] = mulmod(__ldg(in3 + (ct * 3 + 2) * pw + lw), P->inv_qhat[i], P->tab[i].mod);
}

struct DigitMap {
    int D;
    unsigned char prime[32];
    unsigned char shift[32];
};

template <int LOGN>
__global__ void __launch_bounds__(NttPlan<LOGN>::THREADS, NttPlan<LOGN>::MIN_CTAS)
ntt_fwd_digits_kernel(const DeviceParams *__restrict__ P, const uint64_t *__restrict__ dsc, DigitMap map, uint64_t mask,
                      uint64_t *__restrict__ dig) {
    extern __shared__ uint64_t sm[];
    constexpr int N = 1 << LOGN;
    const int K = P->K;
    const long b = blockIdx.x;
    const int j = (int)(b % K);
    const int d = (int)((b / K) % map.D);
    const long ct = b / ((long)K * map.D);
    const NttTable tb = P->tab[j];
    const uint64_t *src = dsc + (ct * K + map.prime[d]) * N;
    const int shift = map.shift[d];
    for (int e = threadIdx.x; e < N; e += blockDim.x) sm[ntt_pad(e)] = (__ldg(src + e) >> shift) & mask;
    __syncthreads();
    ntt_forward_in_smem<LOGN>(sm, tb);
    smem_store_poly_canonical<LOGN>(sm, dig + b * N, tb.mod);
}

__global__ void __launch_bounds__(256)
relin_mac_kernel(const DeviceParams *__restrict__ P, const uint64_t *__restrict__ dig, const uint64_t *__restrict__ evk,
                 RelinArgs a, DigitMap map, uint64_t *__restrict__ acc_out) {
    const int n = P->n, K = P->K;
    const long pw = (long)K * n;
    const long ct = blockIdx.x;
    const long lw = (long)blockIdx.y * 256 + threadIdx.x;
    const int j = (int)(lw / n);
    Acc7 acc0 = acc7_zero(), acc1 = acc7_zero();
    const uint64_t *dp = dig + ct * map.D * pw + lw;
    for (int d = 0; d < map.D; d++) {
        const int i = map.prime[d], k = map.shift[d] / a.dbc;
        const uint64_t *key = evk + a.key_off[i] + (long)(2 * k) * pw + lw;
        const uint64_t dv = __ldg(dp + (long)d * pw);
        mac7(acc0, dv, __ldg(key));
        mac7(acc1, dv, __ldg(key + pw));
    }
    const Mod mod = P->tab[j].mod;
    acc_out[(ct * 2) * pw + lw] = barrett128(acc7_value(acc0), mod);
    acc_out[(ct * 2 + 1) * pw + lw] = barrett128(acc7_value(acc1), mod);
}

__global__ void __launch_bounds__(256)
relin_add_kernel(const DeviceParams *__restrict__ P, const uint64_t *__restrict__ in3, const uint64_t *__restrict__ acc,
                 uint64_t *__restrict__ out) {
    const int n = P->n, K = P->K;
    const long pw = (long)K * n;
    const long ct = blockIdx.x;
    const long w = (long)blockIdx.y * 256 + threadIdx.x;
    const uint64_t q = P->tab[(w % pw) / n].mod.q;
    out[ct * 2 * pw + w] = addmod(__ldg(in3 + ct * 3 * pw + w), __ldg(acc + ct * 2 * pw + w), q);
}

template <int LOGN>
static cudaError_t launch_digits_t(const DeviceParams *P, int K, const uint64_t *dsc, const DigitMap &map, uint64_t mask,
                                   long count, uint64_t *dig, cudaStream_t stream) {
    using Pl = NttPlan<LOGN>;
    size_t smem = Pl::SMEM_WORDS * sizeof(uint64_t);
    auto k = ntt_fwd_digits_kernel<LOGN>;
    static DeviceOnce once;
    if (once.first()) {
        cudaFuncSetAttribute(k, cudaFuncAttributeMaxDynamicSharedMemorySize, (int)smem);
        cudaFuncSetAttribute(k, cudaFuncAttributePreferredSharedMemoryCarveout, cudaSharedmemCarveoutMaxShared);
    }
    k<<<(unsigned)(count * map.D * K), Pl::THREADS, smem, stream>>>(P, dsc, map, mask, dig);
    return cudaGetLastError();
}

cudaError_t launch_relin(const DeviceParams *P, int logn, int K, const RelinArgs &a, cudaStream_t stream) {
    if (a.count <= 0) return cudaSuccess;
    const int n = 1 << logn;
    DigitMap map{};
    for (int i = 0; i < K; i++)
        for (int k = 0; k < a.digits[i]; k++) {
            if (map.D >= 32) return cudaErrorInvalidValue;
            map.prime[map.D] = (unsigned char)i;
            map.shift[map.D] = (unsigned char)(k * a.dbc);
            map.D++;
        }
    const uint64_t mask = (1ULL << a.dbc) - 1;
    dim3 g1((unsigned)a.count, (unsigned)((long)K * n / 256));
    relin_scale_kernel<<<g1, 256, 0, stream>>>(P, a.in3, a.dsc);
    cudaError_t e = cudaGetLastError();
    if (e != cudaSuccess) return e;
    switch (logn) {
        case 10: e = launch_digits_t<10>(P, K, a.dsc, map, mask, a.count, a.dig, stream); break;
        case 11: e = launch_digits_t<11>(P, K, a.dsc, map, mask, a.count, a.dig, stream); break;
        case 12: e = launch_digits_t<12>(P, K, a.dsc, map, mask, a.count, a.dig, stream); break;
        case 13: e = launch_digits_t<13>(P, K, a.dsc, map, mask, a.count, a.dig, stream); break;
        case 14: e = launch_digits_t<14>(P, K, a.dsc, map, mask, a.count, a.dig, stream); break;
        default: return cudaErrorInvalidValue;
    }
    if (e != cudaSuccess) return e;
    relin_mac_kernel<<<g1, 256, 0, stream>>>(P, a.dig, a.evk, a, map, a.acc);
    return cudaGetLastError();
}

cudaError_t launch_relin_finish(const DeviceParams *P, int n, int K, const RelinArgs &a, cudaStream_t stream) {
    if (a.count <= 0) return cudaSuccess;
    dim3 g((unsigned)a.count, (unsigned)(2L * K * n / 256));
    relin_add_kernel<<<g, 256, 0, stream>>>(P, a.in3, a.acc, a.out);
    return cudaGetLastError();
}

static int ew_per(int n) { return n % (512 * 4) == 0 ? 4 : (n % (512 * 2) == 0 ? 2 : 1); }

cudaError_t launch_pool(const DeviceParams *P, int n, int K, const uint64_t *in, const int *in_index, int Nout,
                           int R, const uint64_t *scale_ntt, const uint64_t *scale_shoup, bool sum_fits_64, uint64_t *out,
                           cudaStream_t stream, int per_channel, int channels, const uint64_t *sub) {
    if (Nout <= 0) return cudaSuccess;
    const int per = ew_per(n), chunks = (int)(2L * K * n / (512 * per));
    const unsigned grid = (unsigned)((long)Nout * chunks);
    if (sum_fits_64) pool_kernel<true><<<grid, 256, 0, stream>>>(P, in, in_index, R, scale_ntt, scale_shoup, out, chunks, per, per_channel, channels, sub);
    else pool_kernel<false><<<grid, 256, 0, stream>>>(P, in, in_index, R, scale_ntt, scale_shoup, out, chunks, per, per_channel, channels, sub);
    return cudaGetLastError();
}

__global__ void __launch_bounds__(256)
pool_bn_consts_kernel(const DeviceParams *__restrict__ P, const uint64_t *__restrict__ S, const uint64_t *__restrict__ V,
                      const uint64_t *__restrict__ M, long words, uint64_t *__restrict__ C, uint64_t *__restrict__ D) {
    const long w = (long)blockIdx.x * 256 + threadIdx.x;
    if (w >= words) return;
    const long pw = (long)P->K * P->n, lw = w % pw;
    const Mod mod = P->tab[lw / P->n].mod;
    const uint64_t v = __ldg(V + w);
    C[w] = S ? mulmod(__ldg(S + lw), v, mod) : v;
    D[w] = mulmod(__ldg(M + w), v, mod);
}
cudaError_t launch_pool_bn_consts(const DeviceParams *P, const uint64_t *S, const uint64_t *V, const uint64_t *M, long words,
                                  uint64_t *C, uint64_t *D, cudaStream_t stream) {
    if (words <= 0) return cudaSuccess;
    pool_bn_consts_kernel<<<(unsigned)((words + 255) / 256), 256, 0, stream>>>(P, S, V, M, words, C, D);
    return cudaGetLastError();
}

cudaError_t launch_bn(const DeviceParams *P, int n, int K, const uint64_t *in, long count, int per_channel,
                         int channels, const uint64_t *mean_ntt, const uint64_t *invstd_ntt, const uint64_t *invstd_shoup,
                         uint64_t *out, cudaStream_t stream) {
    if (count <= 0) return cudaSuccess;
    const int per = ew_per(n), chunks = (int)(2L * K * n / (512 * per));
    const unsigned grid = (unsigned)(count * chunks);
    bn_kernel<<<grid, 256, 0, stream>>>(P, in, per_channel, channels, mean_ntt, invstd_ntt, invstd_shoup, out, chunks, per);
    return cudaGetLastError();
}

cudaError_t launch_plain_op(const DeviceParams *P, int n, int K, uint64_t *data, long count, int size,
                               const uint64_t *pl, const uint64_t *pl_sh, int op, cudaStream_t stream) {
    if (count <= 0) return cudaSuccess;
    const long active = (long)(op == 0 ? size : 1) * K * n;
    dim3 grid((unsigned)count, (unsigned)((active / 4 + 255) / 256));
    plain_op_kernel<<<grid, 256, 0, stream>>>(P, data, size, pl, pl_sh, op);
    return cudaGetLastError();
}

#define CRCNN_BEHZ_DISPATCH(KERNEL, GRID, ...)                                                                  \
    do {                                                                                                       \
        if (behz_fold_ok(hp)) {                                                                                \
            if (hp.K == 2 && hp.S == 3) KERNEL<2, 3, true><<<GRID, 128, 0, stream>>>(hp, __VA_ARGS__);          \
            else if (hp.K == 4 && hp.S == 5) KERNEL<4, 5, true><<<GRID, 128, 0, stream>>>(hp, __VA_ARGS__);     \
            else if (hp.K == 8 && hp.S == 9) KERNEL<8, 9, true><<<GRID, 128, 0, stream>>>(hp, __VA_ARGS__);     \
            else KERNEL<0, 0, true><<<GRID, 128, 0, stream>>>(hp, __VA_ARGS__);                                 \
        } else {                                                                                               \
            if (hp.K == 2 && hp.S == 3) KERNEL<2, 3, false><<<GRID, 128, 0, stream>>>(hp, __VA_ARGS__);         \
            else if (hp.K == 4 && hp.S == 5) KERNEL<4, 5, false><<<GRID, 128, 0, stream>>>(hp, __VA_ARGS__);    \
            else if (hp.K == 8 && hp.S == 9) KERNEL<8, 9, false><<<GRID, 128, 0, stream>>>(hp, __VA_ARGS__);    \
            else KERNEL<0, 0, false><<<GRID, 128, 0, stream>>>(hp, __VA_ARGS__);                                \
        }                                                                                                      \
    } while (0)

static bool behz_fold_ok(const DeviceParams &hp) {
    static const int env = [] { const char *e = getenv("CRCNN_BEHZ_FOLD"); return e ? atoi(e) : 1; }();
    if (!env) return false;
    for (int i = 0; i < hp.K + hp.S; i++)
        if (!fold128_make(hp.tab[i].mod.q).ok) return false;
    return true;
}

cudaError_t launch_behz_lift(const DeviceParams &hp, int n, const uint64_t *in, const uint64_t *in_ntt, long count, uint64_t *ext,
                                cudaStream_t stream) {
    if (count <= 0) return cudaSuccess;
    const unsigned grid = (unsigned)(count * 2 * (n / 128));
    CRCNN_BEHZ_DISPATCH(behz_lift_kernel, grid, in, in_ntt, ext);
    return cudaGetLastError();
}

cudaError_t launch_behz_floor(const DeviceParams &hp, int n, const uint64_t *prod, long count, uint64_t *out,
                                 cudaStream_t stream) {
    if (count <= 0) return cudaSuccess;
    const unsigned grid = (unsigned)(count * 3 * (n / 128));
    CRCNN_BEHZ_DISPATCH(behz_floor_kernel, grid, prod, out);
    return cudaGetLastError();
}

__global__ void __launch_bounds__(256)
canonicalize_kernel(const DeviceParams *__restrict__ P, uint64_t *__restrict__ data, long words) {
    const long w = (long)blockIdx.x * 256 + threadIdx.x;
    if (w >= words) return;
    const int n = P->n, K = P->K;
    const uint64_t q = P->tab[(w / n) % K].mod.q;
    uint64_t v = data[w];
    v = v >= 2 * q ? v - 2 * q : v;
    data[w] = v >= q ? v - q : v;
}

cudaError_t launch_canonicalize(const DeviceParams *P, uint64_t *data, long words, cudaStream_t stream) {
    if (words <= 0) return cudaSuccess;
    canonicalize_kernel<<<(unsigned)((words + 255) / 256), 256, 0, stream>>>(P, data, words);
    return cudaGetLastError();
}

__global__ void __launch_bounds__(256)
strip_pad_kernel(const uint64_t *__restrict__ src, uint64_t *__restrict__ dst, int n) {
    const long row = blockIdx.x;
    const uint64_t *s = src + row * (n + 1);
    uint64_t *d = dst + row * n;
    for (int i = threadIdx.x; i < n; i += 256) d[i] = __ldg(s + i);
}

cudaError_t launch_strip_pad(const uint64_t *src_padded, uint64_t *dst, long rows, int n, cudaStream_t stream) {
    if (rows <= 0) return cudaSuccess;
    strip_pad_kernel<<<(unsigned)rows, 256, 0, stream>>>(src_padded, dst, n);
    return cudaGetLastError();
}

__global__ void imad_probe_kernel(int iters, uint64_t *sink) {
    uint64_t a = 0x9E3779B97F4A7C15ULL * (threadIdx.x + 1), b = 0xD1B54A32D192ED03ULL + blockIdx.x;
    Acc7 acc[8];
#pragma unroll
    for (int i = 0; i < 8; i++) acc[i] = acc7_from((uint64_t)i);
    for (int it = 0; it < iters; it++) {
#pragma unroll
        for (int i = 0; i < 8; i++) mac7(acc[i], a + i, b);
        a += acc[0].a3;
        b ^= acc[7].a0;
    }
    uint64_t s = 0;
#pragma unroll
    for (int i = 0; i < 8; i++) { U128 v = acc7_value(acc[i]); s += v.lo ^ v.hi; }
    if (s == 0x1234567) sink[0] = s;
}

cudaError_t launch_imad_probe(int blocks, int threads, int iters, uint64_t *sink, cudaStream_t stream) {
    imad_probe_kernel<<<blocks, threads, 0, stream>>>(iters, sink);
    return cudaGetLastError();
}

__global__ void imad_wide_probe_kernel(int iters, uint64_t *sink) {
    uint32_t a = 0x9E3779B9u * (threadIdx.x + 1), b = 0x85EBCA6Bu + blockIdx.x;
    uint64_t acc[16];
#pragma unroll
    for (int i = 0; i < 16; i++) acc[i] = (uint64_t)i * 0x100000001ull;
    for (int it = 0; it < iters; it++) {
#pragma unroll
        for (int i = 0; i < 16; i++)
            asm volatile("mad.wide.u32 %0, %1, %2, %0;" : "+l"(acc[i]) : "r"(a + i), "r"(b));
    }
    uint64_t s = 0;
#pragma unroll
    for (int i = 0; i < 16; i++) s ^= acc[i];
    if (s == 0x1234567) sink[0] = s;
}

cudaError_t launch_imad_wide_probe(int blocks, int threads, int iters, uint64_t *sink, cudaStream_t stream) {
    imad_wide_probe_kernel<<<blocks, threads, 0, stream>>>(iters, sink);
    return cudaGetLastError();
}

}
```

### crcnn_b200/csrc/kernels.cuh

```cuda
#pragma once
#include <cuda_runtime.h>
#include <cstdint>
#include "params.h"

namespace crcnn {

cudaError_t launch_ntt(const DeviceParams *P, int logn, uint64_t *data, long npolys, int slot_base, int slot_count,
                       bool inverse, cudaStream_t stream);

cudaError_t launch_ntt_grouped(const DeviceParams *P, int logn, uint64_t *data, long npolys, int slot_base, int slot_count,
                               bool inverse, int group_polys, int group_off, cudaStream_t stream, const uint64_t *src = nullptr,
                               const uint64_t *addend = nullptr, int add_group = 1, int add_stride = 1);

cudaError_t launch_plain_expand(const DeviceParams *P, int logn, int K, const uint32_t *offsets, const uint32_t *idx,
                                const uint64_t *val, long first, long count, int mode, bool to_ntt, uint64_t *out,
                                cudaStream_t stream);

struct MacArgs {
    const uint64_t *x;
    const uint64_t *w;
    const uint64_t *bias;
    const int *in_index;
    uint64_t *out;
    int R, M, Npos, Pimg, Mtotal, m0;
    int K, n;
    int chunk_terms;
};
cudaError_t launch_mac(const DeviceParams *P, const MacArgs &a, cudaStream_t stream);

cudaError_t launch_pool(const DeviceParams *P, int n, int K, const uint64_t *in, const int *in_index, int Nout, int R,
                        const uint64_t *scale_ntt, const uint64_t *scale_shoup, bool sum_fits_64, uint64_t *out,
                        cudaStream_t stream, int per_channel = 1, int channels = 0, const uint64_t *sub = nullptr);
cudaError_t launch_pool_bn_consts(const DeviceParams *P, const uint64_t *S, const uint64_t *V, const uint64_t *M, long words,
                                  uint64_t *C, uint64_t *D, cudaStream_t stream);

cudaError_t launch_bn(const DeviceParams *P, int n, int K, const uint64_t *in, long count, int per_channel, int channels,
                      const uint64_t *mean_ntt, const uint64_t *invstd_ntt, const uint64_t *invstd_shoup, uint64_t *out,
                      cudaStream_t stream);

struct TapMulArgs {
    const uint64_t *in;
    const int *in_index;
    int R;
    const uint64_t *sub;
    const uint32_t *t_off;
    const uint32_t *t_idx;
    const uint64_t *t_val;
    int per_channel, channels;
    uint64_t *out;
    long nout;
};
cudaError_t launch_tapmul(const DeviceParams *P, int n, int K, const TapMulArgs &a, cudaStream_t stream);

cudaError_t launch_fold_affine(const DeviceParams *P, uint64_t *data, long rows, long poly_words, int group, const uint64_t *C,
                               const uint64_t *D, cudaStream_t stream);
cudaError_t launch_fold_fc_input_affine(const DeviceParams *P, uint64_t *W, int out_dim, int in_dim, long poly_words, int per_channel,
                                        const uint64_t *C, const uint64_t *D, uint64_t *Bias, cudaStream_t stream);
cudaError_t launch_scale_small(const DeviceParams *P, uint64_t *data, long words, int times, cudaStream_t stream);
cudaError_t launch_shoup_companion(const DeviceParams *P, const uint64_t *data, long words, uint64_t *out, cudaStream_t stream);

cudaError_t launch_plain_op(const DeviceParams *P, int n, int K, uint64_t *data, long count, int size, const uint64_t *pl, const uint64_t *pl_sh, int op,
                            cudaStream_t stream);

cudaError_t launch_behz_lift(const DeviceParams &hp, int n, const uint64_t *in, const uint64_t *in_ntt, long count, uint64_t *ext,
                             cudaStream_t stream);
cudaError_t launch_behz_floor(const DeviceParams &hp, int n, const uint64_t *prod, long count, uint64_t *out, cudaStream_t stream);

struct RelinArgs {
    const uint64_t *in3;
    const uint64_t *evk;
    long key_off[MAXK];
    int digits[MAXK];
    int dbc;
    uint64_t *out;
    long count;
    uint64_t *dsc, *dig, *acc;
};
cudaError_t launch_ntt_inv_tensor(const DeviceParams *P, int logn, const uint64_t *ext, const uint64_t *qntt, long count, int KS, uint64_t *prod,
                                  cudaStream_t stream);

cudaError_t launch_relin(const DeviceParams *P, int logn, int K, const RelinArgs &a, cudaStream_t stream);
cudaError_t launch_relin_finish(const DeviceParams *P, int n, int K, const RelinArgs &a, cudaStream_t stream);

cudaError_t launch_canonicalize(const DeviceParams *P, uint64_t *data, long words, cudaStream_t stream);

cudaError_t launch_strip_pad(const uint64_t *src_padded, uint64_t *dst, long rows, int n, cudaStream_t stream);

cudaError_t launch_imad_probe(int blocks, int threads, int iters, uint64_t *sink, cudaStream_t stream);
cudaError_t launch_imad_wide_probe(int blocks, int threads, int iters, uint64_t *sink, cudaStream_t stream);

}
```

### crcnn_b200/csrc/modarith.cuh

```cuda
#pragma once
#include <cstdint>

#if defined(__CUDACC__)
#define CRCNN_HD __host__ __device__ __forceinline__
#else
#define CRCNN_HD inline
#endif

namespace crcnn {

struct Mod {
    uint64_t q;
    uint64_t r0;
    uint64_t r1;
};

CRCNN_HD uint64_t mulhi64(uint64_t a, uint64_t b) {
#if defined(__CUDA_ARCH__)
    return __umul64hi(a, b);
#else
    return (uint64_t)(((unsigned __int128)a * b) >> 64);
#endif
}

struct U128 {
    uint64_t lo, hi;
};

CRCNN_HD U128 mul128(uint64_t a, uint64_t b) {
    U128 r;
    r.lo = a * b;
    r.hi = mulhi64(a, b);
    return r;
}

CRCNN_HD void mac128(U128 &acc, uint64_t a, uint64_t b) {
    uint64_t lo = a * b;
    uint64_t hi = mulhi64(a, b);
    acc.lo += lo;
    acc.hi += hi + (acc.lo < lo);
}

struct Acc7 {
    uint32_t a0, a1, a2, a3;
    uint32_t b0, b1, b2;
};

CRCNN_HD Acc7 acc7_zero() { return Acc7{0, 0, 0, 0, 0, 0, 0}; }

CRCNN_HD void mac7(Acc7 &c, uint64_t x, uint64_t w) {
#if defined(__CUDA_ARCH__)
    uint32_t x0 = (uint32_t)x, x1 = (uint32_t)(x >> 32), w0 = (uint32_t)w, w1 = (uint32_t)(w >> 32);
    asm("mad.lo.cc.u32 %0, %7, %9, %0;\n\t"
        "madc.hi.cc.u32 %1, %7, %9, %1;\n\t"
        "madc.lo.cc.u32 %2, %8, %10, %2;\n\t"
        "madc.hi.u32 %3, %8, %10, %3;\n\t"
        "mad.lo.cc.u32 %4, %7, %10, %4;\n\t"
        "madc.hi.cc.u32 %5, %7, %10, %5;\n\t"
        "addc.u32 %6, %6, 0;\n\t"
        "mad.lo.cc.u32 %4, %8, %9, %4;\n\t"
        "madc.hi.cc.u32 %5, %8, %9, %5;\n\t"
        "addc.u32 %6, %6, 0;\n\t"
        : "+r"(c.a0), "+r"(c.a1), "+r"(c.a2), "+r"(c.a3), "+r"(c.b0), "+r"(c.b1), "+r"(c.b2)
        : "r"(x0), "r"(x1), "r"(w0), "r"(w1));
#else
    typedef unsigned __int128 u128;
    uint64_t x0 = (uint32_t)x, x1 = x >> 32, w0 = (uint32_t)w, w1 = w >> 32;
    u128 even = ((u128)(((uint64_t)c.a3 << 32) | c.a2) << 64) | (((uint64_t)c.a1 << 32) | c.a0);
    even += (u128)(x0 * w0) + ((u128)(x1 * w1) << 64);
    u128 odd = ((u128)c.b2 << 64) | (((uint64_t)c.b1 << 32) | c.b0);
    odd += (u128)(x0 * w1) + (u128)(x1 * w0);
    c.a0 = (uint32_t)even; c.a1 = (uint32_t)(even >> 32); c.a2 = (uint32_t)(even >> 64); c.a3 = (uint32_t)(even >> 96);
    c.b0 = (uint32_t)odd; c.b1 = (uint32_t)(odd >> 32); c.b2 = (uint32_t)(odd >> 64);
#endif
}

CRCNN_HD U128 acc7_value(const Acc7 &c) {
    uint64_t lo = ((uint64_t)c.a1 << 32) | c.a0, hi = ((uint64_t)c.a3 << 32) | c.a2;
    uint64_t add_lo = (uint64_t)c.b0 << 32, add_hi = ((uint64_t)c.b2 << 32) | c.b1;
    U128 r;
    r.lo = lo + add_lo;
    r.hi = hi + add_hi + (r.lo < lo);
    return r;
}

CRCNN_HD Acc7 acc7_from(uint64_t v) { return Acc7{(uint32_t)v, (uint32_t)(v >> 32), 0, 0, 0, 0, 0}; }

CRCNN_HD void add128_64(U128 &acc, uint64_t v) {
    acc.lo += v;
    acc.hi += (acc.lo < v);
}

CRCNN_HD uint64_t barrett128(U128 z, const Mod &m) {
    uint64_t carry = mulhi64(z.lo, m.r0);
    uint64_t t_lo = z.lo * m.r1;
    uint64_t t_hi = mulhi64(z.lo, m.r1);
    uint64_t s1 = t_lo + carry;
    uint64_t c1 = t_hi + (s1 < carry);
    uint64_t u_lo = z.hi * m.r0;
    uint64_t u_hi = mulhi64(z.hi, m.r0);
    uint64_t s2 = s1 + u_lo;
    uint64_t c2 = u_hi + (s2 < u_lo);
    uint64_t qest = z.hi * m.r1 + c1 + c2;
    uint64_t r = z.lo - qest * m.q;
    return r >= m.q ? r - m.q : r;
}

CRCNN_HD uint64_t reduce64(uint64_t x, const Mod &m) {
    uint64_t r = x - mulhi64(x, m.r1) * m.q;
    return r >= m.q ? r - m.q : r;
}

CRCNN_HD uint64_t mulmod(uint64_t a, uint64_t b, const Mod &m) { return barrett128(mul128(a, b), m); }

CRCNN_HD uint64_t addmod(uint64_t a, uint64_t b, uint64_t q) {
    uint64_t s = a + b;
    return s >= q ? s - q : s;
}
CRCNN_HD uint64_t submod(uint64_t a, uint64_t b, uint64_t q) { return a >= b ? a - b : a + q - b; }
CRCNN_HD uint64_t negmod(uint64_t a, uint64_t q) { return a ? q - a : 0; }

CRCNN_HD uint64_t mulshoup_lazy(uint64_t y, uint64_t w, uint64_t wp, uint64_t q) {
    uint64_t h = mulhi64(wp, y);
    return y * w - h * q;
}

CRCNN_HD uint64_t mulshoup_lazy4(uint64_t y, uint64_t w, uint64_t wp, uint64_t nq) {
#if defined(__CUDA_ARCH__)
    uint32_t y0 = (uint32_t)y, y1 = (uint32_t)(y >> 32), p0 = (uint32_t)wp, p1 = (uint32_t)(wp >> 32);
    uint32_t w0 = (uint32_t)w, w1 = (uint32_t)(w >> 32), n0 = (uint32_t)nq, n1 = (uint32_t)(nq >> 32);
    uint32_t a, b, h0, h1, r0, r1;
    asm("mul.hi.u32 %0, %2, %3;\n\t"
        "mul.hi.u32 %1, %4, %5;\n\t"
        : "=r"(a), "=r"(b) : "r"(p1), "r"(y0), "r"(p0), "r"(y1));
    asm("mad.lo.cc.u32 %0, %2, %3, %4;\n\t"
        "madc.hi.u32 %1, %2, %3, 0;\n\t"
        "add.cc.u32 %0, %0, %5;\n\t"
        "addc.u32 %1, %1, 0;\n\t"
        : "=r"(h0), "=r"(h1) : "r"(p1), "r"(y1), "r"(a), "r"(b));
    asm("mul.lo.u32 %0, %2, %3;\n\t"
        "mul.hi.u32 %1, %2, %3;\n\t"
        "mad.lo.cc.u32 %0, %4, %5, %0;\n\t"
        "madc.hi.u32 %1, %4, %5, %1;\n\t"
        "mad.lo.u32 %1, %2, %6, %1;\n\t"
        "mad.lo.u32 %1, %7, %3, %1;\n\t"
        "mad.lo.u32 %1, %4, %8, %1;\n\t"
        "mad.lo.u32 %1, %9, %5, %1;\n\t"
        : "=&r"(r0), "=&r"(r1) : "r"(y0), "r"(w0), "r"(h0), "r"(n0), "r"(w1), "r"(y1), "r"(n1), "r"(h1));
    return ((uint64_t)r1 << 32) | r0;
#else
    uint64_t y0 = (uint32_t)y, y1 = y >> 32, p0 = (uint32_t)wp, p1 = wp >> 32;
    uint64_t h = p1 * y1 + ((p1 * y0) >> 32) + ((p0 * y1) >> 32);
    return y * w + h * nq;
#endif
}

struct TcnFold {
    uint32_t T;
    uint32_t delta;
    uint32_t sh, mask;
    uint32_t c8, c16, c24;
    uint32_t ok;
};

inline TcnFold tcn_fold_make(uint64_t q) {
    typedef unsigned __int128 u128;
    TcnFold f{};
    int k = 0;
    for (uint64_t v = q; v; v >>= 1) k++;
    if (k < 48 || k > 56) return f;
    const uint64_t delta = (1ull << k) - q;
    if (delta == 0 || delta >> 28) return f;
    const u128 T = (u128)delta << (56 - k);
    if (T >> 32 || T >= q) return f;
    const u128 one = 1, smax = 0x7fffffffu, w32 = 0xffffffffu;
    const u128 La = smax * (1 + (one << 8) + (one << 16) + (one << 24)), Lb = smax * (1 + (one << 8) + (one << 16));
    const u128 Ha = La, Hb = smax * (1 + (one << 8));
    const u128 a = w32 * T + La, b = (Ha >> 32) * T + Lb + w32 * T, e = (Hb >> 32) * T;
    if (a >> 64 || b >> 64 || e >> 60) return f;
    const u128 y = a + (b << 32) + (e << 64);
    const u128 h1 = (y >> k) >> 32;
    const u128 v = w32 * delta + ((one << k) - 1) + (q - 1), w = h1 * delta;
    if (h1 >> 32 || v >> 64 || w >> 62) return f;
    const u128 V = v + (w << 32);
    const u128 g = V >> k;
    if (V >> 96 || g >> 32) return f;
    if (g * delta + ((one << k) - 1) >= 2 * (u128)q) return f;
    f.T = (uint32_t)T; f.delta = (uint32_t)delta; f.sh = (uint32_t)(k - 32); f.mask = (1u << (k - 32)) - 1;
    f.c8 = 1u << 8; f.c16 = 1u << 16; f.c24 = 1u << 24; f.ok = 1;
    return f;
}

CRCNN_HD uint32_t tcn_shr64(uint32_t lo, uint32_t hi, uint32_t sh) {
#if defined(__CUDA_ARCH__)
    return __funnelshift_r(lo, hi, sh);
#else
    return (lo >> sh) | (hi << (32 - sh));
#endif
}

CRCNN_HD uint64_t tcn_fold_reduce(const uint32_t (&s)[13], uint64_t bias, const TcnFold &f, uint64_t q) {
    const uint64_t La = (uint64_t)s[3] * f.c24 + ((uint64_t)s[2] * f.c16 + ((uint64_t)s[1] * f.c8 + s[0]));
    const uint64_t Lb = (uint64_t)s[6] * f.c16 + ((uint64_t)s[5] * f.c8 + s[4]);
    const uint64_t Ha = (uint64_t)s[10] * f.c24 + ((uint64_t)s[9] * f.c16 + ((uint64_t)s[8] * f.c8 + s[7]));
    const uint64_t Hb = (uint64_t)s[12] * f.c8 + s[11];
    const uint64_t a = (uint64_t)(uint32_t)Ha * f.T + La;
    const uint64_t b = (uint64_t)(uint32_t)Hb * f.T + ((Ha >> 32) * f.T + Lb);
    const uint64_t e = (Hb >> 32) * f.T;
    const uint32_t y0 = (uint32_t)a;
    const uint64_t m1 = (a >> 32) + (uint32_t)b;
    const uint32_t y1 = (uint32_t)m1;
    const uint64_t m2 = (b >> 32) + (uint64_t)(uint32_t)e + (m1 >> 32);
    const uint32_t y2 = (uint32_t)m2;
    const uint32_t y3 = (uint32_t)(e >> 32) + (uint32_t)(m2 >> 32);
    const uint32_t h0 = tcn_shr64(y1, y2, f.sh), h1 = tcn_shr64(y2, y3, f.sh);
    const uint64_t l = ((uint64_t)(y1 & f.mask) << 32) | y0;
    const uint64_t v = (uint64_t)h0 * f.delta + l + bias;
    const uint64_t w = (uint64_t)h1 * f.delta;
    const uint64_t m3 = (v >> 32) + (uint32_t)w;
    const uint32_t V1 = (uint32_t)m3, V2 = (uint32_t)(w >> 32) + (uint32_t)(m3 >> 32);
    const uint32_t g = tcn_shr64(V1, V2, f.sh);
    const uint64_t lo = ((uint64_t)(V1 & f.mask) << 32) | (uint32_t)v;
    const uint64_t r = (uint64_t)g * f.delta + lo;
    return r >= q ? r - q : r;
}

struct Fold128 {
    uint64_t q;
    uint32_t delta, sh, mask, ok;
};

inline Fold128 fold128_make(uint64_t q) {
    typedef unsigned __int128 u128;
    Fold128 f{};
    f.q = q;
    int k = 0;
    for (uint64_t v = q; v; v >>= 1) k++;
    if (k < 54 || k > 61) return f;
    const uint64_t delta = (1ull << k) - q;
    if (delta == 0 || delta >> 27) return f;
    const u128 one = 1, zmax = ~(u128)0;
    const u128 y = ((one << k) - 1) + (zmax >> k) * delta;
    const u128 V = ((one << k) - 1) + (y >> k) * delta;
    const u128 g = V >> k;
    if (y >> 112 || (y >> k) >> 64 || V >> 96 || g >> 32) return f;
    if (g * delta + ((one << k) - 1) >= 2 * (u128)q) return f;
    f.delta = (uint32_t)delta; f.sh = (uint32_t)(k - 32); f.mask = (1u << (k - 32)) - 1; f.ok = 1;
    return f;
}

CRCNN_HD uint64_t reduce128_fold(U128 z, const Fold128 &f) {
    const uint32_t z0 = (uint32_t)z.lo, z1 = (uint32_t)(z.lo >> 32), z2 = (uint32_t)z.hi, z3 = (uint32_t)(z.hi >> 32);
    const uint32_t h0 = tcn_shr64(z1, z2, f.sh), h1 = tcn_shr64(z2, z3, f.sh), h2 = z3 >> f.sh;
    const uint64_t l = ((uint64_t)(z1 & f.mask) << 32) | z0;
    const uint64_t t0 = (uint64_t)h0 * f.delta + l;
    const uint64_t u = (uint64_t)h1 * f.delta + (t0 >> 32);
    const uint64_t u2 = (uint64_t)h2 * f.delta + (u >> 32);
    const uint32_t y0 = (uint32_t)t0, y1 = (uint32_t)u, y2 = (uint32_t)u2, y3 = (uint32_t)(u2 >> 32);
    const uint32_t g0 = tcn_shr64(y1, y2, f.sh), g1 = tcn_shr64(y2, y3, f.sh);
    const uint64_t l2 = ((uint64_t)(y1 & f.mask) << 32) | y0;
    const uint64_t v = (uint64_t)g0 * f.delta + l2;
    const uint64_t w = (uint64_t)g1 * f.delta + (v >> 32);
    const uint32_t V0 = (uint32_t)v, V1 = (uint32_t)w, V2 = (uint32_t)(w >> 32);
    const uint32_t g = tcn_shr64(V1, V2, f.sh);
    const uint64_t l3 = ((uint64_t)(V1 & f.mask) << 32) | V0;
    const uint64_t r = (uint64_t)g * f.delta + l3;
    return r >= f.q ? r - f.q : r;
}

}
```

### crcnn_b200/csrc/ntt.cuh

```cuda
#pragma once
#include "modarith.cuh"
#include "params.h"

namespace crcnn {

__device__ __forceinline__ int ntt_pad(int i) { return i + ((i >> 4) << 1); }

template <int LOGN>
struct NttPlan {
    static constexpr int N = 1 << LOGN;
    static constexpr int THREADS = N / 32;
    static constexpr int SMEM_WORDS = N + N / 8;
    static constexpr int FIT = (227 * 1024) / (SMEM_WORDS * 8);
    static constexpr int MIN_CTAS = FIT > 768 / THREADS ? 768 / THREADS : (FIT < 1 ? 1 : FIT);
    static constexpr int PASSES = (LOGN + 3) / 4;
    static constexpr int WIDE = LOGN - 3 * PASSES;
    __host__ __device__ static constexpr int bits(int pass) { return pass >= PASSES - WIDE ? 4 : 3; }
    __host__ __device__ static constexpr int skip_passes() {
        int st = 0, p = 0;
        while (st < sparse_skip_stages(LOGN)) { st += bits(p); p++; }
        return p;
    }
};

__device__ __forceinline__ bool ntt_needs_correction(uint64_t q) { return (q >> 57) != 0; }
__device__ __forceinline__ int ntt_fwd_mode(uint64_t q) { return (q >> 57) == 0 ? 0 : ((q >> 61) == 0 ? 2 : 1); }
__device__ __forceinline__ bool ntt_inv_exact(uint64_t q) { return (q >> 61) != 0; }

template <int MODE>
__device__ __forceinline__ void ct_butterfly(uint64_t &x, uint64_t &y, uint64_t W, uint64_t Wp, uint64_t c, uint64_t c2) {
    if (MODE == 1) {
        uint64_t X = x >= c2 ? x - c2 : x;
        uint64_t Q = mulshoup_lazy(y, W, Wp, c);
        x = X + Q;
        y = X + c2 - Q;
    } else if (MODE == 2) {
        uint64_t X = x >= c2 ? x - c2 : x;
        uint64_t Q = mulshoup_lazy4(y, W, Wp, c);
        x = X + Q;
        y = X + c2 - Q;
    } else {
        uint64_t Q = mulshoup_lazy4(y, W, Wp, c);
        uint64_t X = x;
        x = X + Q;
        y = X + c2 - Q;
    }
}

template <bool CORR>
__device__ __forceinline__ void gs_butterfly(uint64_t &u, uint64_t &v, uint64_t W, uint64_t Wp, uint64_t c, uint64_t c2) {
    if (CORR) {
        uint64_t T = u + c2 - v;
        uint64_t S = u + v;
        u = S >= c2 ? S - c2 : S;
        v = mulshoup_lazy(T, W, Wp, c);
    } else {
        uint64_t T = u + c2 - v;
        uint64_t S = u + v;
        u = S >= c2 ? S - c2 : S;
        v = mulshoup_lazy4(T, W, Wp, c);
    }
}

template <int B, int CORR>
__device__ __forceinline__ void fwd_group(uint64_t (&x)[1 << B], const ulonglong2 *__restrict__ w,
                                          uint64_t q, uint64_t twoq, int m0, int blk) {
#pragma unroll
    for (int s = 0; s < B; s++) {
#pragma unroll
        for (int pr = 0; pr < (1 << (B - 1)); pr++) {
            const int lb = pr >> (B - 1 - s), a = pr & ((1 << (B - 1 - s)) - 1);
            const int ia = (lb << (B - s)) + a, ib = ia + (1 << (B - 1 - s));
            const int tw = ((m0 + blk) << s) + lb;
            const ulonglong2 W = __ldg(w + tw);
            ct_butterfly<CORR>(x[ia], x[ib], W.x, W.y, q, twoq);
        }
    }
}

template <int B, bool CORR>
__device__ __forceinline__ void inv_group(uint64_t (&x)[1 << B], const ulonglong2 *__restrict__ iw,
                                          uint64_t q, uint64_t twoq, int h0, int blk) {
#pragma unroll
    for (int s = 0; s < B; s++) {
#pragma unroll
        for (int pr = 0; pr < (1 << (B - 1)); pr++) {
            const int lb = pr >> s, a = pr & ((1 << s) - 1);
            const int ia = (lb << (s + 1)) + a, ib = ia + (1 << s);
            const int tw = (h0 >> s) + (blk << (B - 1 - s)) + lb;
            const ulonglong2 W = __ldg(iw + tw);
            gs_butterfly<CORR>(x[ia], x[ib], W.x, W.y, q, twoq);
        }
    }
}

template <int LOGN, int B, bool SRC_GLOBAL, int CORR>
__device__ __forceinline__ void fwd_pass(uint64_t *sm, const uint64_t *__restrict__ gsrc, const NttTable &tb, int m0, int g) {
    constexpr int N = 1 << LOGN;
    const uint64_t q = CORR == 1 ? tb.mod.q : 0 - tb.mod.q, twoq = CORR == 1 ? 2 * tb.mod.q : 4 * tb.mod.q;
    for (int G = threadIdx.x; G < (N >> B); G += blockDim.x) {
        int blk = G / g, o = G - blk * g;
        int base = blk * (g << B) + o;
        uint64_t x[1 << B];
#pragma unroll
        for (int k = 0; k < (1 << B); k++) x[k] = SRC_GLOBAL ? gsrc[base + k * g] : sm[ntt_pad(base + k * g)];
        fwd_group<B, CORR>(x, reinterpret_cast<const ulonglong2 *>(tb.w), q, twoq, m0, blk);
#pragma unroll
        for (int k = 0; k < (1 << B); k++) sm[ntt_pad(base + k * g)] = x[k];
    }
}

template <int LOGN, int CORR>
__device__ __forceinline__ void fwd_last_pass(uint64_t *sm, const NttTable &tb) {
    constexpr int N = 1 << LOGN, NG = N >> 4;
    const uint64_t q = CORR == 1 ? tb.mod.q : 0 - tb.mod.q, twoq = CORR == 1 ? 2 * tb.mod.q : 4 * tb.mod.q;
    const ulonglong2 *wl = reinterpret_cast<const ulonglong2 *>(tb.wl);
    for (int G = threadIdx.x; G < NG; G += blockDim.x) {
        ulonglong2 *row = reinterpret_cast<ulonglong2 *>(sm + 18 * G);
        uint64_t x[16];
#pragma unroll
        for (int m = 0; m < 8; m++) {
            const ulonglong2 v = row[m];
            x[2 * m] = v.x;
            x[2 * m + 1] = v.y;
        }
#pragma unroll
        for (int s = 0; s < 4; s++) {
#pragma unroll
            for (int lb = 0; lb < (1 << s); lb++) {
                const ulonglong2 W = __ldg(wl + ((1 << s) - 1 + lb) * NG + G);
#pragma unroll
                for (int a = 0; a < (1 << (3 - s)); a++) {
                    const int ia = (lb << (4 - s)) + a;
                    ct_butterfly<CORR>(x[ia], x[ia + (1 << (3 - s))], W.x, W.y, q, twoq);
                }
            }
        }
#pragma unroll
        for (int m = 0; m < 8; m++) row[m] = make_ulonglong2(x[2 * m], x[2 * m + 1]);
    }
}

template <int LOGN, bool CORR>
__device__ __forceinline__ void inv_first_pass(uint64_t *sm, const NttTable &tb) {
    constexpr int N = 1 << LOGN, NG = N >> 4;
    const uint64_t q = tb.mod.q;
    const uint64_t c = CORR ? q : 0 - q, c2 = CORR ? 2 * q : 4 * q;
    const ulonglong2 *iwl = reinterpret_cast<const ulonglong2 *>(tb.iwl);
    for (int G = threadIdx.x; G < NG; G += blockDim.x) {
        ulonglong2 *row = reinterpret_cast<ulonglong2 *>(sm + 18 * G);
        uint64_t x[16];
#pragma unroll
        for (int m = 0; m < 8; m++) {
            const ulonglong2 v = row[m];
            x[2 * m] = v.x;
            x[2 * m + 1] = v.y;
        }
#pragma unroll
        for (int s = 0; s < 4; s++) {
#pragma unroll
            for (int lb = 0; lb < (1 << (3 - s)); lb++) {
                const ulonglong2 W = __ldg(iwl + (16 - (16 >> s) + lb) * NG + G);
#pragma unroll
                for (int a = 0; a < (1 << s); a++) {
                    const int ia = (lb << (s + 1)) + a;
                    gs_butterfly<CORR>(x[ia], x[ia + (1 << s)], W.x, W.y, c, c2);
                }
            }
        }
#pragma unroll
        for (int m = 0; m < 8; m++) row[m] = make_ulonglong2(x[2 * m], x[2 * m + 1]);
    }
}

template <int LOGN, int B, bool DST_GLOBAL, bool CORR>
__device__ __forceinline__ void inv_pass(uint64_t *sm, uint64_t *__restrict__ gdst, const NttTable &tb, int g,
                                         const uint64_t *__restrict__ gadd = nullptr) {
    constexpr int N = 1 << LOGN;
    const uint64_t q = tb.mod.q;
    const uint64_t c = CORR ? q : 0 - q, c2 = CORR ? 2 * q : 4 * q;
    const int h0 = N / (2 * g);
    for (int G = threadIdx.x; G < (N >> B); G += blockDim.x) {
        int blk = G / g, o = G - blk * g;
        int base = blk * (g << B) + o;
        uint64_t x[1 << B];
#pragma unroll
        for (int k = 0; k < (1 << B); k++) x[k] = sm[ntt_pad(base + k * g)];
        inv_group<B, CORR>(x, reinterpret_cast<const ulonglong2 *>(tb.iw), c, c2, h0, blk);
#pragma unroll
        for (int k = 0; k < (1 << B); k++) {
            if (DST_GLOBAL) {
                uint64_t v = mulshoup_lazy(x[k], tb.ninv, tb.ninvp, q);
                v = v >= q ? v - q : v;
                if (gadd) v = addmod(v, __ldg(gadd + base + k * g), q);
                gdst[base + k * g] = v;
            } else {
                sm[ntt_pad(base + k * g)] = x[k];
            }
        }
    }
}

template <int LOGN, int FIRST_PASS, int CORR>
__device__ __forceinline__ void ntt_forward_passes(uint64_t *sm, const uint64_t *__restrict__ src, const NttTable &tb) {
    using P = NttPlan<LOGN>;
    int m0 = 1, g = P::N;
#pragma unroll
    for (int p = 0; p < FIRST_PASS; p++) { g >>= P::bits(p); m0 <<= P::bits(p); }
#pragma unroll
    for (int p = FIRST_PASS; p < P::PASSES; p++) {
        g >>= P::bits(p);
        if (p == P::PASSES - 1 && P::bits(p) == 4 && !(p == 0 && src != nullptr)) {
            fwd_last_pass<LOGN, CORR>(sm, tb);
        } else if (p == 0 && src != nullptr) {
            if (P::bits(p) == 4) fwd_pass<LOGN, 4, true, CORR>(sm, src, tb, m0, g); else fwd_pass<LOGN, 3, true, CORR>(sm, src, tb, m0, g);
        } else {
            if (P::bits(p) == 4) fwd_pass<LOGN, 4, false, CORR>(sm, nullptr, tb, m0, g); else fwd_pass<LOGN, 3, false, CORR>(sm, nullptr, tb, m0, g);
        }
        m0 <<= P::bits(p);
        __syncthreads();
    }
}

template <int LOGN>
__device__ __forceinline__ void ntt_forward_to_smem(uint64_t *sm, const uint64_t *__restrict__ src, const NttTable &tb) {
    const int mode = ntt_fwd_mode(tb.mod.q);
    if (mode == 0) ntt_forward_passes<LOGN, 0, 0>(sm, src, tb);
    else if (mode == 2) ntt_forward_passes<LOGN, 0, 2>(sm, src, tb);
    else ntt_forward_passes<LOGN, 0, 1>(sm, src, tb);
}

template <int LOGN, int FIRST_PASS = 0>
__device__ __forceinline__ void ntt_forward_in_smem(uint64_t *sm, const NttTable &tb) {
    const int mode = ntt_fwd_mode(tb.mod.q);
    if (mode == 0) ntt_forward_passes<LOGN, FIRST_PASS, 0>(sm, nullptr, tb);
    else if (mode == 2) ntt_forward_passes<LOGN, FIRST_PASS, 2>(sm, nullptr, tb);
    else ntt_forward_passes<LOGN, FIRST_PASS, 1>(sm, nullptr, tb);
}

template <int LOGN, bool CORR>
__device__ __forceinline__ void ntt_inverse_passes(uint64_t *sm, uint64_t *__restrict__ dst, const NttTable &tb,
                                                   const uint64_t *__restrict__ add) {
    using P = NttPlan<LOGN>;
    int g = 1;
#pragma unroll
    for (int p = P::PASSES - 1; p >= 1; p--) {
        if (p == P::PASSES - 1 && P::bits(p) == 4) inv_first_pass<LOGN, CORR>(sm, tb);
        else if (P::bits(p) == 4) inv_pass<LOGN, 4, false, CORR>(sm, nullptr, tb, g); else inv_pass<LOGN, 3, false, CORR>(sm, nullptr, tb, g);
        g <<= P::bits(p);
        __syncthreads();
    }
    if (P::bits(0) == 4) inv_pass<LOGN, 4, true, CORR>(sm, dst, tb, g, add); else inv_pass<LOGN, 3, true, CORR>(sm, dst, tb, g, add);
}

template <int LOGN>
__device__ __forceinline__ void ntt_inverse_from_smem(uint64_t *sm, uint64_t *__restrict__ dst, const NttTable &tb,
                                                      const uint64_t *__restrict__ add = nullptr) {
    if (ntt_inv_exact(tb.mod.q)) ntt_inverse_passes<LOGN, true>(sm, dst, tb, add);
    else ntt_inverse_passes<LOGN, false>(sm, dst, tb, add);
}

template <int LOGN>
__device__ __forceinline__ void smem_load_poly(uint64_t *sm, const uint64_t *__restrict__ src) {
#pragma unroll 8
    for (int i = threadIdx.x; i < (1 << LOGN); i += NttPlan<LOGN>::THREADS) sm[ntt_pad(i)] = src[i];
}
template <int LOGN>
__device__ __forceinline__ void smem_store_poly_canonical(const uint64_t *sm, uint64_t *__restrict__ dst, const Mod &mod) {
#pragma unroll 8
    for (int i = threadIdx.x; i < (1 << LOGN); i += NttPlan<LOGN>::THREADS) dst[i] = reduce64(sm[ntt_pad(i)], mod);
}

}
```

### crcnn_b200/csrc/params.cpp

```cpp
#include "params.h"
#include <cmath>
#include <stdexcept>

namespace crcnn {

typedef unsigned __int128 u128;

static const uint64_t kAuxPrimes[] = {
    0x1fffffffffb40001ULL, 0x1fffffffff500001ULL, 0x1fffffffff380001ULL, 0x1fffffffff000001ULL,
    0x1ffffffffef00001ULL, 0x1ffffffffee80001ULL, 0x1ffffffffeb40001ULL, 0x1ffffffffe780001ULL,
    0x1ffffffffe600001ULL, 0x1ffffffffe4c0001ULL};
static const uint64_t kMsk = 0x1fffffffffe00001ULL;
static const uint64_t kMtilde = 1ULL << 32;

static int bits_of(uint64_t v) {
    int b = 0;
    for (; v; v >>= 1) b++;
    return b;
}

Mod make_mod(uint64_t q) {
    u128 ones = ~(u128)0;
    u128 quo = ones / q;
    if (ones % q == (u128)(q - 1)) quo++;
// ... 18 lines not shown
    __int128 r0 = q, r1 = a % q, s0 = 0, s1 = 1;
    while (r1 != 0) {
        __int128 k = r0 / r1;
        __int128 r2 = r0 - k * r1, s2 = s0 - k * s1;
        r0 = r1; r1 = r2; s0 = s1; s1 = s2;
    }
    if (r0 != 1) throw std::invalid_argument("inv_mod: operand not invertible");
    if (s0 < 0) s0 += q;
    return (uint64_t)s0;
}

bool minimal_primitive_root(uint64_t degree, const Mod &m, uint64_t &root) {
    if ((m.q - 1) % degree) return false;
    uint64_t cof = (m.q - 1) / degree, start = 0;
    for (uint64_t g = 2; g < 1u << 16 && !start; g++) {
        uint64_t c = pow_mod(g, cof, m);
        if (pow_mod(c, degree / 2, m) == m.q - 1) start = c;
    }
    if (!start) return false;
    uint64_t step = mulmod(start, start, m), cur = start, best = start;
    for (uint64_t i = 0; i < degree / 2; i++) {
        if (cur < best) best = cur;
        cur = mulmod(cur, step, m);
    }
    root = best;
    return true;
}

static uint32_t bit_reverse(uint32_t x, int bits) {
    uint32_t r = 0;
    for (int i = 0; i < bits; i++, x >>= 1) r = (r << 1) | (x & 1);
    return r;
}

static uint64_t product_mod(const uint64_t *v, int count, int skip, const Mod &m) {
    uint64_t r = 1 % m.q;
    for (int i = 0; i < count; i++)
        if (i != skip) r = mulmod(r, v[i] % m.q, m);
    return r;
}

static void build_tables(HostParams &hp, int slot, int logn, const Mod &m) {
    int n = 1 << logn;
    uint64_t psi;
    if (!minimal_primitive_root(2ull * n, m, psi))
        throw std::invalid_argument("modulus " + std::to_string(m.q) + " has no primitive 2n-th root of unity");
    uint64_t psi_inv = inv_mod(psi, m.q);
    auto &w = hp.w[slot], &wp = hp.wp[slot], &iw = hp.iw[slot], &iwp = hp.iwp[slot];
    auto &iwf = hp.iwf[slot], &iwfp = hp.iwfp[slot];
    w.assign(n, 0); wp.assign(n, 0); iw.assign(n, 0); iwp.assign(n, 0); iwf.assign(n, 0); iwfp.assign(n, 0);
    uint64_t pw = 1, ipw = 1;
    for (int i = 0; i < n; i++) {
        uint32_t r = bit_reverse((uint32_t)i, logn);
        w[r] = pw;
        iw[r] = (ipw & 1) ? (uint64_t)(((u128)ipw + m.q) >> 1) : (ipw >> 1);
        iwf[r] = ipw;
        pw = mulmod(pw, psi, m);
        ipw = mulmod(ipw, psi_inv, m);
    }
    for (int i = 0; i < n; i++) {
        wp[i] = (uint64_t)((((u128)w[i]) << 64) / m.q);
        iwp[i] = (uint64_t)((((u128)iw[i]) << 64) / m.q);
        iwfp[i] = (uint64_t)((((u128)iwf[i]) << 64) / m.q);
    }
    hp.d.tab[slot].ninv = inv_mod((uint64_t)n % m.q, m.q);
    hp.d.tab[slot].ninvp = (uint64_t)((((u128)hp.d.tab[slot].ninv) << 64) / m.q);
    hp.roots[slot] = psi;
}

HostParams derive_params(int n, int K, const uint64_t *q, uint64_t t) {
    int logn = 0;
    while ((1 << logn) < n) logn++;
    if (n < 1024 || n > 16384 || (1 << logn) != n) throw std::invalid_argument("n must be a power of two in [1024, 16384]");
    if (K < 1 || K > MAXK) throw std::invalid_argument("coefficient modulus count must be in [1, 8]");
    if (t < 2) throw std::invalid_argument("plain modulus must be at least 2");
    int total_bits = 0;
    for (int i = 0; i < K; i++) {
        if (bits_of(q[i]) > 60 || q[i] < 2) throw std::invalid_argument("coefficient primes must be at most 60 bits");
        if (q[i] <= t) throw std::invalid_argument("plain modulus must be smaller than every coefficient prime (fast plain lift)");
        for (int j = 0; j < i; j++)
            if (q[i] == q[j]) throw std::invalid_argument("coefficient primes must be distinct");
        total_bits += bits_of(q[i]);
    }
    HostParams hp;
    DeviceParams &d = hp.d;
    d.n = n; d.logn = logn; d.K = K; d.t = t; d.half = (t + 1) >> 1;
    d.L = K + ((32 + bits_of(t) + total_bits >= 61 * K + 61) ? 1 : 0);
    d.S = d.L + 1;
    int slots = K + d.S;
    hp.w.resize(slots); hp.wp.resize(slots); hp.iw.resize(slots); hp.iwp.resize(slots); hp.iwf.resize(slots); hp.iwfp.resize(slots); hp.roots.resize(slots);

    std::vector<uint64_t> bsk(d.S);
    for (int i = 0; i < d.L; i++) bsk[i] = kAuxPrimes[i];
    bsk[d.L] = kMsk;
    for (int i = 0; i < K; i++) { d.tab[i].mod = make_mod(q[i]); build_tables(hp, i, logn, d.tab[i].mod); }
    for (int k = 0; k < d.S; k++) { d.tab[K + k].mod = make_mod(bsk[k]); build_tables(hp, K + k, logn, d.tab[K + k].mod); }
    for (int s = 0; s < slots; s++) d.t_mod[s] = t % d.tab[s].mod.q;
    hp.tf.resize(K);
    const int skip = sparse_skip_stages(logn);
    for (int j = 0; j < K; j++) {
        const Mod &m = d.tab[j].mod;
        hp.tf[j].assign((size_t)1 << skip, 0);
        for (int b = 0; b < (1 << skip); b++) {
            uint64_t c = 1;
            for (int s = 0; s < skip; s++) {
                uint64_t w = hp.w[j][((size_t)1 << s) + (b >> (skip - s))];
                if ((b >> (skip - 1 - s)) & 1) w = negmod(w, m.q);
                c = mulmod(c, w, m);
            }
            hp.tf[j][b] = c;
        }
    }

    Mod mt = make_mod(kMtilde), msk = make_mod(kMsk), tm = make_mod(t);
    uint64_t rho = product_mod(q, K, -1, tm);
    for (int j = 0; j < K; j++) {
        const Mod &m = d.tab[j].mod;
        d.rho[j] = rho % m.q;
        d.delta[j] = mulmod(negmod(d.rho[j], m.q), inv_mod(t % m.q, m.q), m);
        d.lift_inc[j] = m.q - t;
        d.inv_qhat[j] = inv_mod(product_mod(q, K, j, m), m.q);
        d.mt_inv_qhat[j] = mulmod(d.inv_qhat[j], kMtilde % m.q, m);
        d.qhat_mod_mt[j] = product_mod(q, K, j, mt);
        d.M_mod_q[j] = product_mod(bsk.data(), d.L, -1, m);
        d.neg_M_mod_q[j] = m.q - d.M_mod_q[j];
        for (int i = 0; i < d.L; i++) d.Mhat_mod_q[j][i] = product_mod(bsk.data(), d.L, i, m);
    }
    d.neg_inv_q_mod_mt = (kMtilde - inv_mod(product_mod(q, K, -1, mt), kMtilde)) % kMtilde;
    for (int k = 0; k < d.S; k++) {
        const Mod &m = d.tab[K + k].mod;
        for (int i = 0; i < K; i++) d.qhat_mod_bsk[k][i] = product_mod(q, K, i, m);
        d.q_mod_bsk[k] = product_mod(q, K, -1, m);
        d.inv_q_mod_bsk[k] = inv_mod(d.q_mod_bsk[k], m.q);
        d.inv_mt_mod_bsk[k] = inv_mod(kMtilde % m.q, m.q);
    }
    for (int i = 0; i < d.L; i++) {
        const Mod &m = d.tab[K + i].mod;
        d.inv_Mhat[i] = inv_mod(product_mod(bsk.data(), d.L, i, m), m.q);
        d.Mhat_mod_msk[i] = product_mod(bsk.data(), d.L, i, msk);
    }
    d.inv_M_mod_msk = inv_mod(product_mod(bsk.data(), d.L, -1, msk), kMsk);
    for (int j = 0; j < K; j++) d.fl_c[j] = mulmod(t % d.tab[j].mod.q, d.inv_qhat[j], d.tab[j].mod);
    for (int k = 0; k < d.S; k++) {
        const Mod &m = d.tab[K + k].mod;
        const uint64_t fold = k < d.L ? mulmod(d.inv_q_mod_bsk[k], d.inv_Mhat[k], m) : d.inv_q_mod_bsk[k];
        d.lift_b[k] = mulmod(d.q_mod_bsk[k], d.inv_mt_mod_bsk[k], m);
        d.fl_T[k] = mulmod(t % m.q, fold, m);
        for (int i = 0; i < K; i++) {
            d.lift_a[k][i] = mulmod(d.qhat_mod_bsk[k][i], d.inv_mt_mod_bsk[k], m);
            d.fl_N[k][i] = negmod(mulmod(d.qhat_mod_bsk[k][i], fold, m), m.q);
        }
    }
    for (int i = 0; i < d.L; i++) d.fl_P[i] = mulmod(d.Mhat_mod_msk[i], d.inv_M_mod_msk, msk);
    return hp;
}

static void encode_integer_b3(int64_t v, uint64_t t, std::vector<uint32_t> &idx, std::vector<uint64_t> &val) {
    bool neg = v < 0;
    uint64_t mag = neg ? (uint64_t)(-v) : (uint64_t)v;
    for (uint32_t pos = 0; mag; pos++) {
        uint64_t rem = mag % 3;
        int digit = rem == 0 ? 0 : (rem == 1 ? 1 : -1);
        mag = (mag + 1) / 3;
        if (neg) digit = -digit;
        if (digit) { idx.push_back(pos); val.push_back(digit > 0 ? 1 : t - 1); }
    }
}

void encode_fractional_sparse(double value, int n, uint64_t t, std::vector<uint32_t> &idx,
                              std::vector<uint64_t> &val) {
    int64_t ip = (int64_t)std::round(value);
    encode_integer_b3(ip, t, idx, val);
    double frac = value - (double)ip;
    if (frac == 0) return;
    for (int i = 0; i < 32; i++) {
        frac *= 3.0;
        int sign = frac >= 0 ? 1 : -1;
        int64_t digit = (int64_t)(sign * std::ceil(std::fabs(frac) - 0.5));
        frac -= (double)digit;
        if (digit) { idx.push_back((uint32_t)(n - 1 - i)); val.push_back(digit > 0 ? t - (uint64_t)digit : (uint64_t)(-digit)); }
    }
}

}
```

### crcnn_b200/csrc/params.h

```cpp
#pragma once
#include <cstdint>
#include <string>
#include <vector>
#include "modarith.cuh"

namespace crcnn {

constexpr int MAXK = 8;
constexpr int MAXS = 10;
constexpr int MAXDIG = 4;

struct NttTable {
    Mod mod;
    const uint64_t *w;
    const uint64_t *iw;
    uint64_t ninv, ninvp;
    const uint64_t *tf;
    const uint64_t *wl;
    const uint64_t *iwl;
};

#if defined(__CUDACC__)
__host__ __device__
#endif
constexpr int sparse_skip_stages(int logn) { return logn == 13 ? 6 : logn == 12 ? 4 : logn == 14 ? 6 : 3; }

struct DeviceParams {
    int n, logn, K, L, S;
    uint64_t t, half;
    NttTable tab[MAXK + MAXS];
    uint64_t delta[MAXK];
    uint64_t rho[MAXK];
    uint64_t lift_inc[MAXK];
    uint64_t inv_qhat[MAXK];
    uint64_t mt_inv_qhat[MAXK];
    uint64_t qhat_mod_bsk[MAXS][MAXK];
    uint64_t qhat_mod_mt[MAXK];
    uint64_t neg_inv_q_mod_mt;
    uint64_t q_mod_bsk[MAXS];
    uint64_t inv_mt_mod_bsk[MAXS];
    uint64_t inv_q_mod_bsk[MAXS];
    uint64_t inv_Mhat[MAXS];
    uint64_t Mhat_mod_q[MAXK][MAXS];
    uint64_t Mhat_mod_msk[MAXS];
    uint64_t inv_M_mod_msk;
    uint64_t M_mod_q[MAXK];
    uint64_t neg_M_mod_q[MAXK];
    uint64_t t_mod[MAXK + MAXS];
    uint64_t lift_a[MAXS][MAXK];
    uint64_t lift_b[MAXS];
    uint64_t fl_c[MAXK];
    uint64_t fl_T[MAXS];
    uint64_t fl_N[MAXS][MAXK];
    uint64_t fl_P[MAXS];
};

struct HostParams {
    DeviceParams d{};
    std::vector<std::vector<uint64_t>> w, wp, iw, iwp;
    std::vector<std::vector<uint64_t>> iwf, iwfp;
    std::vector<uint64_t> roots;
    std::vector<std::vector<uint64_t>> tf;
};

HostParams derive_params(int n, int K, const uint64_t *q, uint64_t t);

Mod make_mod(uint64_t q);
uint64_t inv_mod(uint64_t a, uint64_t q);
uint64_t pow_mod(uint64_t a, uint64_t e, const Mod &m);
bool minimal_primitive_root(uint64_t degree, const Mod &m, uint64_t &root);

void encode_fractional_sparse(double value, int n, uint64_t t, std::vector<uint32_t> &idx,
                              std::vector<uint64_t> &val);

}
```

Measured before the change: 38.28.

## Fold n^-1 scaling into BEHZ constants and use fold reduction in square path

Adds a lean square path that skips the n^-1 multiply at the end of the inverse NTTs. The scaling is absorbed into precomputed BEHZ lift/floor constants (mt_inv_qhat_n, fl_c_n, fl_T_n). The tensor kernel uses a pseudo-Mersenne fold reduction instead of Barrett when the moduli allow it. It also adds a shape-specialised 64-bit reduce for canonical stores, a dedicated squaring routine, and a mul.wide tweak in the lazy Shoup multiply. This saves modular multiplies per coefficient across several kernels, at the cost of more template variants and a new invariant: the later floor and lift stages must know their inputs are unscaled.

```diff
diff --git a/crcnn_b200/csrc/engine.cu b/crcnn_b200/csrc/engine.cu
--- a/crcnn_b200/csrc/engine.cu
+++ b/crcnn_b200/csrc/engine.cu
@@ -99,6 +99,7 @@
     int tap_mode = 1;
     int relin_mode = 1;
     int tcn_mode = 1;
+    int sq_lean = 1;
     int tcn_fold = 1;
     size_t tc_scratch_bytes = 12ull << 30;
     std::string err;
@@ -578,6 +579,7 @@
     if (const char *e = getenv("CRCNN_TCN")) c->tcn_mode = atoi(e);
     if (const char *e = getenv("CRCNN_TAP")) c->tap_mode = atoi(e);
     if (const char *e = getenv("CRCNN_TCN_FOLD")) c->tcn_fold = atoi(e);
+    if (const char *e = getenv("CRCNN_SQ_LEAN")) c->sq_lean = atoi(e);
     cudaMemPool_t pool;
     if (cudaDeviceGetDefaultMemPool(&pool, device) == cudaSuccess) {
         uint64_t thr = UINT64_MAX;
@@ -1486,6 +1488,7 @@
     REQUIRE(in->size == 2, "square expects size-2 ciphertexts");
     CU(cudaSetDevice(ctx->device));
     const bool have_ntt = in->ntt != 0;
+    const bool lean = ctx->sq_lean != 0, fold = lean && behz_fold_ok(ctx->hp.d), copy_ninv = !(lean && have_ntt);
     crcnn_tensor *o = nullptr;
     int rc = new_tensor(ctx, in->count, 3, 0, &o);
     if (rc) return rc;
@@ -1503,9 +1506,10 @@
         cudaError_t e = cudaSuccess;
         if (have_ntt) {
             ProfScope ps(ctx, KC_NTT_INV, 2 * lp_bytes(ctx, (double)cur * 2 * ctx->K), lp_bfly(ctx, (double)cur * 2 * ctx->K));
-            e = launch_ntt_grouped(ctx->dP, ctx->logn, coef, cur * 2 * ctx->K, 0, ctx->K, true, ctx->K, 0, ctx->stream, src);
+            e = launch_ntt_grouped(ctx->dP, ctx->logn, coef, cur * 2 * ctx->K, 0, ctx->K, true, ctx->K, 0, ctx->stream, src,
+                                   nullptr, 1, 1, copy_ninv);
         }
-        if (e == cudaSuccess) { ProfScope ps(ctx, KC_BEHZ_LIFT, lp_bytes(ctx, (double)cur * 2 * (ctx->K + (have_ntt ? ctx->S : KS))), (double)cur * 2 * n * ctx->S * (ctx->K + 1)); e = launch_behz_lift(ctx->hp.d, ctx->n, have_ntt ? coef : src, have_ntt ? src : nullptr, cur, ext, ctx->stream); }
+        if (e == cudaSuccess) { ProfScope ps(ctx, KC_BEHZ_LIFT, lp_bytes(ctx, (double)cur * 2 * (ctx->K + (have_ntt ? ctx->S : KS))), (double)cur * 2 * n * ctx->S * (ctx->K + 1)); e = launch_behz_lift(ctx->hp.d, ctx->n, have_ntt ? coef : src, have_ntt ? src : nullptr, cur, ext, ctx->stream, copy_ninv); }
         if (e == cudaSuccess) {
             if (have_ntt) {
                 ProfScope ps(ctx, KC_NTT_FWD, 2 * lp_bytes(ctx, (double)cur * 2 * ctx->S), lp_bfly(ctx, (double)cur * 2 * ctx->S));
@@ -1517,10 +1521,10 @@
         }
         if (e == cudaSuccess) {
             ProfScope ps(ctx, KC_SQ_TENSOR, lp_bytes(ctx, (double)cur * 5 * KS), lp_bfly(ctx, (double)cur * 3 * KS));
-            e = launch_ntt_inv_tensor(ctx->dP, ctx->logn, ext, have_ntt ? src : nullptr, cur, KS, prod, ctx->stream);
+            e = launch_ntt_inv_tensor(ctx->dP, ctx->logn, ext, have_ntt ? src : nullptr, cur, KS, prod, fold, !lean, ctx->stream);
         }
         if (e == cudaSuccess) { ProfScope ps(ctx, KC_BEHZ_FLOOR, lp_bytes(ctx, (double)cur * 3 * (KS + ctx->K)),
-                                                     (double)cur * 3 * n * (ctx->S * (ctx->K + 1) + ctx->S + ctx->K * ctx->S)); e = launch_behz_floor(ctx->hp.d, ctx->n, prod, cur, o->d + c0 * 3 * pw, ctx->stream); }
+                                                     (double)cur * 3 * n * (ctx->S * (ctx->K + 1) + ctx->S + ctx->K * ctx->S)); e = launch_behz_floor(ctx->hp.d, ctx->n, prod, cur, o->d + c0 * 3 * pw, ctx->stream, !lean); }
         if (e != cudaSuccess) rc = fail(ctx, CRCNN_ERR_CUDA, cudaGetErrorString(e));
     }
     dev_free(ctx, coef);
diff --git a/crcnn_b200/csrc/host_selftest.cpp b/crcnn_b200/csrc/host_selftest.cpp
--- a/crcnn_b200/csrc/host_selftest.cpp
+++ b/crcnn_b200/csrc/host_selftest.cpp
@@ -80,6 +80,54 @@
                 if (reduce128_fold(z, f) != want || barrett128(z, m) != want) { printf("FOLD128 MISMATCH\n"); return 1; }
             }
         }
+        typedef unsigned __int128 u128;
+        for (int s = 0; s < d.K + d.S; s++) {
+            const uint64_t q = d.tab[s].mod.q;
+            const bool ok_ninv = (u128)d.tab[s].ninv * (uint64_t)n % q == 1;
+            bool ok = ok_ninv;
+            if (s < d.K) {
+                ok = ok && d.mt_inv_qhat_n[s] < q && (u128)d.mt_inv_qhat_n[s] * (uint64_t)n % q == d.mt_inv_qhat[s];
+                ok = ok && d.fl_c_n[s] < q && (u128)d.fl_c_n[s] * (uint64_t)n % q == d.fl_c[s];
+            } else {
+                ok = ok && d.fl_T_n[s - d.K] < q && (u128)d.fl_T_n[s - d.K] * (uint64_t)n % q == d.fl_T[s - d.K];
+            }
+            printf("ninv %d ok %d\n", s, ok ? 1 : 0);
+            if (!ok) { printf("NINV CONSTANT MISMATCH\n"); return 1; }
+        }
+        for (int s = 0; s < d.K + d.S; s++) {
+            const uint64_t q = d.tab[s].mod.q, nq = 0 - q;
+            const uint64_t ws[] = {0, 1, q - 1, q / 2, 0x5555555555555555ULL % q, 0};
+            long checked = 0;
+            for (int wi = 0; wi < 6; wi++) {
+                uint64_t w = ws[wi];
+                for (int it = 0; it < 20000; it++) {
+                    x = x * 6364136223846793005ULL + 1442695040888963407ULL;
+                    y = y * 2862933555777941757ULL + 3037000493ULL;
+                    if (wi == 5) w = y % q;
+                    const uint64_t wp = (uint64_t)(((u128)w << 64) / q);
+                    const int mode = it % 8;
+                    const uint64_t yv = mode == 0 ? 0 : mode == 1 ? ~0ull : mode == 2 ? (x % (~0ull / q + 1)) * q
+                                      : mode == 3 ? (~0ull / q) * q : mode == 4 ? q - 1 : mode == 5 ? 8 * q - 1 - (x & 7) : x;
+                    const uint64_t r = mulshoup_lazy4(yv, w, wp, nq);
+                    if (r >= 4 * q || r % q != (uint64_t)((u128)w * yv % q)) { printf("SHOUP4 MISMATCH\n"); return 1; }
+                    const uint64_t a = x % q;
+                    const U128 z = sqr128(a);
+                    if (((u128)z.hi << 64 | z.lo) != (u128)a * a) { printf("SQR128 MISMATCH\n"); return 1; }
+                    checked++;
+                }
+            }
+            printf("shoup4 %d checked %ld\n", s, checked);
+            const int k = reduce64_shape_k(q);
+            if (k) {
+                for (int it = 0; it < 200000; it++) {
+                    x = x * 6364136223846793005ULL + 1442695040888963407ULL;
+                    const int mode = it % 6;
+                    const uint64_t v = mode == 0 ? ~0ull : mode == 1 ? 0 : mode == 2 ? q : mode == 3 ? q - 1 : mode == 4 ? (x % 16) * q + (x >> 60) : x;
+                    if (reduce64_shape(v, q, k) != v % q || reduce64(v, d.tab[s].mod) != v % q) { printf("REDUCE64 MISMATCH\n"); return 1; }
+                }
+            }
+            printf("reduce64_shape %d k %d\n", s, k);
+        }
         for (int i = 4; i >= 0; i--) {
             double vals[] = {0.0867, -3.25, 0.0, 1.0, 2.8215};
             std::vector<uint32_t> idx; std::vector<uint64_t> val;
diff --git a/crcnn_b200/csrc/kernels.cu b/crcnn_b200/csrc/kernels.cu
--- a/crcnn_b200/csrc/kernels.cu
+++ b/crcnn_b200/csrc/kernels.cu
@@ -2,6 +2,7 @@
 #include "devcfg.cuh"
 #include "ntt.cuh"
 #include <cstdlib>
+#include <cstring>
 
 namespace crcnn {
 
@@ -17,7 +18,7 @@
     smem_store_poly_canonical<LOGN>(sm, poly, tb.mod);
 }
 
-template <int LOGN>
+template <int LOGN, bool NINV>
 __global__ void __launch_bounds__(NttPlan<LOGN>::THREADS, NttPlan<LOGN>::MIN_CTAS)
 ntt_inv_kernel(uint64_t *__restrict__ data, const DeviceParams *__restrict__ P, int slot_base, int slot_count, int group_polys,
                int group_off, const uint64_t *__restrict__ src, const uint64_t *__restrict__ addend, int add_group, int add_stride) {
@@ -28,10 +29,24 @@
     uint64_t *poly = data + off;
     smem_load_poly<LOGN>(sm, src ? src + off : poly);
     __syncthreads();
-    ntt_inverse_from_smem<LOGN>(sm, poly, tb, addend ? addend + ((p / add_group) * add_stride + p % add_group) * (1L << LOGN) : nullptr);
-}
-
-template <int LOGN>
+    ntt_inverse_from_smem<LOGN, NINV>(sm, poly, tb, addend ? addend + ((p / add_group) * add_stride + p % add_group) * (1L << LOGN) : nullptr);
+}
+
+template <bool FOLD>
+__device__ __forceinline__ uint64_t behz_reduce(U128 z, const Mod &m) {
+    if constexpr (FOLD) {
+        Fold128 f;
+        const int k = 64 - __clzll((long long)m.q);
+        f.q = m.q; f.delta = (uint32_t)((1ull << k) - m.q); f.sh = (uint32_t)(k - 32); f.mask = (1u << (k - 32)) - 1; f.ok = 1;
+        return reduce128_fold(z, f);
+    } else {
+        return barrett128(z, m);
+    }
+}
+template <bool FOLD>
+__device__ __forceinline__ uint64_t behz_mulmod(uint64_t a, uint64_t b, const Mod &m) { return behz_reduce<FOLD>(mul128(a, b), m); }
+
+template <int LOGN, bool FOLD, bool NINV>
 __global__ void __launch_bounds__(NttPlan<LOGN>::THREADS, NttPlan<LOGN>::MIN_CTAS)
 ntt_inv_tensor_kernel(const DeviceParams *__restrict__ P, const uint64_t *__restrict__ ext, const uint64_t *__restrict__ qntt, int KS,
                       uint64_t *__restrict__ prod) {
@@ -50,27 +65,34 @@
     if (k == 1) {
 #pragma unroll 8
         for (int i = threadIdx.x; i < N; i += NttPlan<LOGN>::THREADS) {
-            const uint64_t ab = mulmod(__ldg(c0 + i), __ldg(c1 + i), tb.mod);
-            sm[ntt_pad(i)] = addmod(ab, ab, tb.mod.q);
+            if (FOLD) {
+                U128 z = mul128(__ldg(c0 + i), __ldg(c1 + i));
+                z.hi = (z.hi << 1) | (z.lo >> 63);
+                z.lo <<= 1;
+                sm[ntt_pad(i)] = behz_reduce<true>(z, tb.mod);
+            } else {
+                const uint64_t ab = mulmod(__ldg(c0 + i), __ldg(c1 + i), tb.mod);
+                sm[ntt_pad(i)] = addmod(ab, ab, tb.mod.q);
+            }
         }
     } else {
         const uint64_t *c = k == 0 ? c0 : c1;
 #pragma unroll 8
         for (int i = threadIdx.x; i < N; i += NttPlan<LOGN>::THREADS) {
             const uint64_t a = __ldg(c + i);
-            sm[ntt_pad(i)] = mulmod(a, a, tb.mod);
+            sm[ntt_pad(i)] = FOLD ? behz_reduce<true>(sqr128(a), tb.mod) : mulmod(a, a, tb.mod);
         }
     }
     __syncthreads();
-    ntt_inverse_from_smem<LOGN>(sm, prod + b * N, tb);
-}
-
-template <int LOGN>
+    ntt_inverse_from_smem<LOGN, NINV>(sm, prod + b * N, tb);
+}
+
+template <int LOGN, bool FOLD, bool NINV>
 static cudaError_t launch_ntt_inv_tensor_t(const DeviceParams *P, const uint64_t *ext, const uint64_t *qntt, long count, int KS, uint64_t *prod,
                                            cudaStream_t stream) {
     using Pl = NttPlan<LOGN>;
     const size_t smem = Pl::SMEM_WORDS * sizeof(uint64_t);
-    auto kf = ntt_inv_tensor_kernel<LOGN>;
+    auto kf = ntt_inv_tensor_kernel<LOGN, FOLD, NINV>;
     static DeviceOnce once;
     if (once.first()) {
         cudaFuncSetAttribute(kf, cudaFuncAttributeMaxDynamicSharedMemorySize, (int)smem);
@@ -80,15 +102,24 @@
     return cudaGetLastError();
 }
 
+template <int LOGN>
+static cudaError_t launch_ntt_inv_tensor_l(const DeviceParams *P, const uint64_t *ext, const uint64_t *qntt, long count, int KS, uint64_t *prod,
+                                           bool fold, bool ninv, cudaStream_t stream) {
+    if (!ninv) return fold ? launch_ntt_inv_tensor_t<LOGN, true, false>(P, ext, qntt, count, KS, prod, stream)
+                           : launch_ntt_inv_tensor_t<LOGN, false, false>(P, ext, qntt, count, KS, prod, stream);
+    if (fold) return cudaErrorInvalidValue;
+    return launch_ntt_inv_tensor_t<LOGN, false, true>(P, ext, qntt, count, KS, prod, stream);
+}
+
 cudaError_t launch_ntt_inv_tensor(const DeviceParams *P, int logn, const uint64_t *ext, const uint64_t *qntt, long count, int KS, uint64_t *prod,
-                                  cudaStream_t stream) {
+                                  bool fold, bool ninv, cudaStream_t stream) {
     if (count <= 0) return cudaSuccess;
     switch (logn) {
-        case 10: return launch_ntt_inv_tensor_t<10>(P, ext, qntt, count, KS, prod, stream);
-        case 11: return launch_ntt_inv_tensor_t<11>(P, ext, qntt, count, KS, prod, stream);
-        case 12: return launch_ntt_inv_tensor_t<12>(P, ext, qntt, count, KS, prod, stream);
-        case 13: return launch_ntt_inv_tensor_t<13>(P, ext, qntt, count, KS, prod, stream);
-        case 14: return launch_ntt_inv_tensor_t<14>(P, ext, qntt, count, KS, prod, stream);
+        case 10: return launch_ntt_inv_tensor_l<10>(P, ext, qntt, count, KS, prod, fold, ninv, stream);
+        case 11: return launch_ntt_inv_tensor_l<11>(P, ext, qntt, count, KS, prod, fold, ninv, stream);
+        case 12: return launch_ntt_inv_tensor_l<12>(P, ext, qntt, count, KS, prod, fold, ninv, stream);
+        case 13: return launch_ntt_inv_tensor_l<13>(P, ext, qntt, count, KS, prod, fold, ninv, stream);
+        case 14: return launch_ntt_inv_tensor_l<14>(P, ext, qntt, count, KS, prod, fold, ninv, stream);
         default: return cudaErrorInvalidValue;
     }
 }
@@ -96,34 +127,37 @@
 template <int LOGN>
 static cudaError_t launch_ntt_t(const DeviceParams *P, uint64_t *data, long npolys, int slot_base, int slot_count,
                                 bool inverse, int group_polys, int group_off, const uint64_t *src, const uint64_t *addend,
-                                int add_group, int add_stride, cudaStream_t stream) {
+                                int add_group, int add_stride, bool ninv, cudaStream_t stream) {
     using Pl = NttPlan<LOGN>;
     size_t smem = Pl::SMEM_WORDS * sizeof(uint64_t);
     auto kf = ntt_fwd_kernel<LOGN>;
-    auto ki = ntt_inv_kernel<LOGN>;
+    auto ki = ntt_inv_kernel<LOGN, true>;
+    auto kn = ntt_inv_kernel<LOGN, false>;
     static DeviceOnce once;
     if (once.first()) {
         cudaFuncSetAttribute(kf, cudaFuncAttributeMaxDynamicSharedMemorySize, (int)smem);
         cudaFuncSetAttribute(ki, cudaFuncAttributeMaxDynamicSharedMemorySize, (int)smem);
+        cudaFuncSetAttribute(kn, cudaFuncAttributeMaxDynamicSharedMemorySize, (int)smem);
         cudaFuncSetAttribute(kf, cudaFuncAttributePreferredSharedMemoryCarveout, cudaSharedmemCarveoutMaxShared);
         cudaFuncSetAttribute(ki, cudaFuncAttributePreferredSharedMemoryCarveout, cudaSharedmemCarveoutMaxShared);
+        cudaFuncSetAttribute(kn, cudaFuncAttributePreferredSharedMemoryCarveout, cudaSharedmemCarveoutMaxShared);
     }
     if (npolys <= 0) return cudaSuccess;
-    if ((src || addend) && !inverse) return cudaErrorInvalidValue;
-    if (inverse) ki<<<(unsigned)npolys, Pl::THREADS, smem, stream>>>(data, P, slot_base, slot_count, group_polys, group_off, src, addend, add_group, add_stride);
+    if ((src || addend || !ninv) && !inverse) return cudaErrorInvalidValue;
+    if (inverse) (ninv ? ki : kn)<<<(unsigned)npolys, Pl::THREADS, smem, stream>>>(data, P, slot_base, slot_count, group_polys, group_off, src, addend, add_group, add_stride);
     else kf<<<(unsigned)npolys, Pl::THREADS, smem, stream>>>(data, P, slot_base, slot_count, group_polys, group_off);
     return cudaGetLastError();
 }
 
 cudaError_t launch_ntt_grouped(const DeviceParams *P, int logn, uint64_t *data, long npolys, int slot_base, int slot_count,
                                bool inverse, int group_polys, int group_off, cudaStream_t stream, const uint64_t *src,
-                               const uint64_t *addend, int add_group, int add_stride) {
+                               const uint64_t *addend, int add_group, int add_stride, bool ninv) {
     switch (logn) {
-        case 10: return launch_ntt_t<10>(P, data, npolys, slot_base, slot_count, inverse, group_polys, group_off, src, addend, add_group, add_stride, stream);
-        case 11: return launch_ntt_t<11>(P, data, npolys, slot_base, slot_count, inverse, group_polys, group_off, src, addend, add_group, add_stride, stream);
-        case 12: return launch_ntt_t<12>(P, data, npolys, slot_base, slot_count, inverse, group_polys, group_off, src, addend, add_group, add_stride, stream);
-        case 13: return launch_ntt_t<13>(P, data, npolys, slot_base, slot_count, inverse, group_polys, group_off, src, addend, add_group, add_stride, stream);
-        case 14: return launch_ntt_t<14>(P, data, npolys, slot_base, slot_count, inverse, group_polys, group_off, src, addend, add_group, add_stride, stream);
+        case 10: return launch_ntt_t<10>(P, data, npolys, slot_base, slot_count, inverse, group_polys, group_off, src, addend, add_group, add_stride, ninv, stream);
+        case 11: return launch_ntt_t<11>(P, data, npolys, slot_base, slot_count, inverse, group_polys, group_off, src, addend, add_group, add_stride, ninv, stream);
+        case 12: return launch_ntt_t<12>(P, data, npolys, slot_base, slot_count, inverse, group_polys, group_off, src, addend, add_group, add_stride, ninv, stream);
+        case 13: return launch_ntt_t<13>(P, data, npolys, slot_base, slot_count, inverse, group_polys, group_off, src, addend, add_group, add_stride, ninv, stream);
+        case 14: return launch_ntt_t<14>(P, data, npolys, slot_base, slot_count, inverse, group_polys, group_off, src, addend, add_group, add_stride, ninv, stream);
         default: return cudaErrorInvalidValue;
     }
 }
@@ -692,20 +726,6 @@
     x[0] = a; x[1] = b;
 }
 
-template <bool FOLD>
-__device__ __forceinline__ uint64_t behz_reduce(U128 z, const Mod &m) {
-    if constexpr (FOLD) {
-        Fold128 f;
-        const int k = 64 - __clzll((long long)m.q);
-        f.q = m.q; f.delta = (uint32_t)((1ull << k) - m.q); f.sh = (uint32_t)(k - 32); f.mask = (1u << (k - 32)) - 1; f.ok = 1;
-        return reduce128_fold(z, f);
-    } else {
-        return barrett128(z, m);
-    }
-}
-template <bool FOLD>
-__device__ __forceinline__ uint64_t behz_mulmod(uint64_t a, uint64_t b, const Mod &m) { return behz_reduce<FOLD>(mul128(a, b), m); }
-
 template <int KT, int ST, bool FOLD>
 __global__ void __launch_bounds__(128)
 behz_lift_kernel(const __grid_constant__ DeviceParams P, const uint64_t *__restrict__ in, const uint64_t *__restrict__ in_ntt,
@@ -974,7 +994,7 @@
         }                                                                                                      \
     } while (0)
 
-static bool behz_fold_ok(const DeviceParams &hp) {
+bool behz_fold_ok(const DeviceParams &hp) {
     static const int env = [] { const char *e = getenv("CRCNN_BEHZ_FOLD"); return e ? atoi(e) : 1; }();
     if (!env) return false;
     for (int i = 0; i < hp.K + hp.S; i++)
@@ -982,17 +1002,31 @@
     return true;
 }
 
-cudaError_t launch_behz_lift(const DeviceParams &hp, int n, const uint64_t *in, const uint64_t *in_ntt, long count, uint64_t *ext,
-                                cudaStream_t stream) {
+cudaError_t launch_behz_lift(const DeviceParams &P, int n, const uint64_t *in, const uint64_t *in_ntt, long count, uint64_t *ext,
+                                cudaStream_t stream, bool ninv_in) {
     if (count <= 0) return cudaSuccess;
+    if (!ninv_in && !in_ntt) return cudaErrorInvalidValue;
+    DeviceParams scaled;
+    if (!ninv_in) {
+        scaled = P;
+        std::memcpy(scaled.mt_inv_qhat, P.mt_inv_qhat_n, sizeof scaled.mt_inv_qhat);
+    }
+    const DeviceParams &hp = ninv_in ? P : scaled;
     const unsigned grid = (unsigned)(count * 2 * (n / 128));
     CRCNN_BEHZ_DISPATCH(behz_lift_kernel, grid, in, in_ntt, ext);
     return cudaGetLastError();
 }
 
-cudaError_t launch_behz_floor(const DeviceParams &hp, int n, const uint64_t *prod, long count, uint64_t *out,
-                                 cudaStream_t stream) {
+cudaError_t launch_behz_floor(const DeviceParams &P, int n, const uint64_t *prod, long count, uint64_t *out,
+                                 cudaStream_t stream, bool ninv_in) {
     if (count <= 0) return cudaSuccess;
+    DeviceParams scaled;
+    if (!ninv_in) {
+        scaled = P;
+        std::memcpy(scaled.fl_c, P.fl_c_n, sizeof scaled.fl_c);
+        std::memcpy(scaled.fl_T, P.fl_T_n, sizeof scaled.fl_T);
+    }
+    const DeviceParams &hp = ninv_in ? P : scaled;
     const unsigned grid = (unsigned)(count * 3 * (n / 128));
     CRCNN_BEHZ_DISPATCH(behz_floor_kernel, grid, prod, out);
     return cudaGetLastError();
diff --git a/crcnn_b200/csrc/kernels.cuh b/crcnn_b200/csrc/kernels.cuh
--- a/crcnn_b200/csrc/kernels.cuh
+++ b/crcnn_b200/csrc/kernels.cuh
@@ -10,7 +10,7 @@
 
 cudaError_t launch_ntt_grouped(const DeviceParams *P, int logn, uint64_t *data, long npolys, int slot_base, int slot_count,
                                bool inverse, int group_polys, int group_off, cudaStream_t stream, const uint64_t *src = nullptr,
-                               const uint64_t *addend = nullptr, int add_group = 1, int add_stride = 1);
+                               const uint64_t *addend = nullptr, int add_group = 1, int add_stride = 1, bool ninv = true);
 
 cudaError_t launch_plain_expand(const DeviceParams *P, int logn, int K, const uint32_t *offsets, const uint32_t *idx,
                                 const uint64_t *val, long first, long count, int mode, bool to_ntt, uint64_t *out,
@@ -63,8 +63,10 @@
                             cudaStream_t stream);
 
 cudaError_t launch_behz_lift(const DeviceParams &hp, int n, const uint64_t *in, const uint64_t *in_ntt, long count, uint64_t *ext,
-                             cudaStream_t stream);
-cudaError_t launch_behz_floor(const DeviceParams &hp, int n, const uint64_t *prod, long count, uint64_t *out, cudaStream_t stream);
+                             cudaStream_t stream, bool ninv_in = true);
+cudaError_t launch_behz_floor(const DeviceParams &hp, int n, const uint64_t *prod, long count, uint64_t *out, cudaStream_t stream,
+                              bool ninv_in = true);
+bool behz_fold_ok(const DeviceParams &hp);
 
 struct RelinArgs {
     const uint64_t *in3;
@@ -77,7 +79,7 @@
     uint64_t *dsc, *dig, *acc;
 };
 cudaError_t launch_ntt_inv_tensor(const DeviceParams *P, int logn, const uint64_t *ext, const uint64_t *qntt, long count, int KS, uint64_t *prod,
-                                  cudaStream_t stream);
+                                  bool fold, bool ninv, cudaStream_t stream);
 
 cudaError_t launch_relin(const DeviceParams *P, int logn, int K, const RelinArgs &a, cudaStream_t stream);
 cudaError_t launch_relin_finish(const DeviceParams *P, int n, int K, const RelinArgs &a, cudaStream_t stream);
diff --git a/crcnn_b200/csrc/modarith.cuh b/crcnn_b200/csrc/modarith.cuh
--- a/crcnn_b200/csrc/modarith.cuh
+++ b/crcnn_b200/csrc/modarith.cuh
@@ -31,6 +31,15 @@
     U128 r;
     r.lo = a * b;
     r.hi = mulhi64(a, b);
+    return r;
+}
+
+CRCNN_HD U128 sqr128(uint64_t a) {
+    const uint64_t a0 = (uint32_t)a, a1 = a >> 32;
+    const uint64_t lo = a0 * a0, mid = (a0 * a1) << 1, hi = a1 * a1;
+    U128 r;
+    r.lo = lo + (mid << 32);
+    r.hi = hi + (mid >> 32) + (r.lo < lo);
     return r;
 }
 
@@ -111,6 +120,17 @@
     return r >= m.q ? r - m.q : r;
 }
 
+CRCNN_HD int reduce64_shape_k(uint64_t q) {
+    int k = 0;
+    for (uint64_t v = q; v; v >>= 1) k++;
+    return (k >= 48 && k <= 63 && ((1ull << k) - q) < (1ull << 27)) ? k : 0;
+}
+CRCNN_HD uint64_t reduce64_shape(uint64_t x, uint64_t q, int k) {
+    const uint32_t delta = (uint32_t)((1ull << k) - q), hi = (uint32_t)(x >> k);
+    const uint64_t r = (x & ((1ull << k) - 1)) + (uint64_t)hi * delta;
+    return r >= q ? r - q : r;
+}
+
 CRCNN_HD uint64_t mulmod(uint64_t a, uint64_t b, const Mod &m) { return barrett128(mul128(a, b), m); }
 
 CRCNN_HD uint64_t addmod(uint64_t a, uint64_t b, uint64_t q) {
@@ -130,9 +150,12 @@
     uint32_t y0 = (uint32_t)y, y1 = (uint32_t)(y >> 32), p0 = (uint32_t)wp, p1 = (uint32_t)(wp >> 32);
     uint32_t w0 = (uint32_t)w, w1 = (uint32_t)(w >> 32), n0 = (uint32_t)nq, n1 = (uint32_t)(nq >> 32);
     uint32_t a, b, h0, h1, r0, r1;
-    asm("mul.hi.u32 %0, %2, %3;\n\t"
-        "mul.hi.u32 %1, %4, %5;\n\t"
-        : "=r"(a), "=r"(b) : "r"(p1), "r"(y0), "r"(p0), "r"(y1));
+    uint64_t wa, wb;
+    asm("mul.wide.u32 %0, %2, %3;\n\t"
+        "mul.wide.u32 %1, %4, %5;\n\t"
+        : "=l"(wa), "=l"(wb) : "r"(p1), "r"(y0), "r"(p0), "r"(y1));
+    a = (uint32_t)(wa >> 32);
+    b = (uint32_t)(wb >> 32);
     asm("mad.lo.cc.u32 %0, %2, %3, %4;\n\t"
         "madc.hi.u32 %1, %2, %3, 0;\n\t"
         "add.cc.u32 %0, %0, %5;\n\t"
diff --git a/crcnn_b200/csrc/ntt.cuh b/crcnn_b200/csrc/ntt.cuh
--- a/crcnn_b200/csrc/ntt.cuh
+++ b/crcnn_b200/csrc/ntt.cuh
@@ -173,7 +173,7 @@
     }
 }
 
-template <int LOGN, int B, bool DST_GLOBAL, bool CORR>
+template <int LOGN, int B, bool DST_GLOBAL, bool CORR, bool NINV = true>
 __device__ __forceinline__ void inv_pass(uint64_t *sm, uint64_t *__restrict__ gdst, const NttTable &tb, int g,
                                          const uint64_t *__restrict__ gadd = nullptr) {
     constexpr int N = 1 << LOGN;
@@ -190,7 +190,12 @@
 #pragma unroll
         for (int k = 0; k < (1 << B); k++) {
             if (DST_GLOBAL) {
-                uint64_t v = mulshoup_lazy(x[k], tb.ninv, tb.ninvp, q);
+                uint64_t v;
+                if (NINV) {
+                    v = mulshoup_lazy(x[k], tb.ninv, tb.ninvp, q);
+                } else {
+                    v = x[k] >= 2 * q ? x[k] - 2 * q : x[k];
+                }
                 v = v >= q ? v - q : v;
                 if (gadd) v = addmod(v, __ldg(gadd + base + k * g), q);
                 gdst[base + k * g] = v;
@@ -238,7 +243,7 @@
     else ntt_forward_passes<LOGN, FIRST_PASS, 1>(sm, nullptr, tb);
 }
 
-template <int LOGN, bool CORR>
+template <int LOGN, bool CORR, bool NINV>
 __device__ __forceinline__ void ntt_inverse_passes(uint64_t *sm, uint64_t *__restrict__ dst, const NttTable &tb,
                                                    const uint64_t *__restrict__ add) {
     using P = NttPlan<LOGN>;
@@ -250,14 +255,14 @@
         g <<= P::bits(p);
         __syncthreads();
     }
-    if (P::bits(0) == 4) inv_pass<LOGN, 4, true, CORR>(sm, dst, tb, g, add); else inv_pass<LOGN, 3, true, CORR>(sm, dst, tb, g, add);
-}
-
-template <int LOGN>
+    if (P::bits(0) == 4) inv_pass<LOGN, 4, true, CORR, NINV>(sm, dst, tb, g, add); else inv_pass<LOGN, 3, true, CORR, NINV>(sm, dst, tb, g, add);
+}
+
+template <int LOGN, bool NINV = true>
 __device__ __forceinline__ void ntt_inverse_from_smem(uint64_t *sm, uint64_t *__restrict__ dst, const NttTable &tb,
                                                       const uint64_t *__restrict__ add = nullptr) {
-    if (ntt_inv_exact(tb.mod.q)) ntt_inverse_passes<LOGN, true>(sm, dst, tb, add);
-    else ntt_inverse_passes<LOGN, false>(sm, dst, tb, add);
+    if (ntt_inv_exact(tb.mod.q)) ntt_inverse_passes<LOGN, true, NINV>(sm, dst, tb, add);
+    else ntt_inverse_passes<LOGN, false, NINV>(sm, dst, tb, add);
 }
 
 template <int LOGN>
@@ -267,8 +272,14 @@
 }
 template <int LOGN>
 __device__ __forceinline__ void smem_store_poly_canonical(const uint64_t *sm, uint64_t *__restrict__ dst, const Mod &mod) {
+    const int k = reduce64_shape_k(mod.q);
+    if (k) {
 #pragma unroll 8
-    for (int i = threadIdx.x; i < (1 << LOGN); i += NttPlan<LOGN>::THREADS) dst[i] = reduce64(sm[ntt_pad(i)], mod);
-}
-
-}
+        for (int i = threadIdx.x; i < (1 << LOGN); i += NttPlan<LOGN>::THREADS) dst[i] = reduce64_shape(sm[ntt_pad(i)], mod.q, k);
+    } else {
+#pragma unroll 8
+        for (int i = threadIdx.x; i < (1 << LOGN); i += NttPlan<LOGN>::THREADS) dst[i] = reduce64(sm[ntt_pad(i)], mod);
+    }
+}
+
+}
diff --git a/crcnn_b200/csrc/params.cpp b/crcnn_b200/csrc/params.cpp
--- a/crcnn_b200/csrc/params.cpp
+++ b/crcnn_b200/csrc/params.cpp
@@ -194,6 +194,11 @@
         }
     }
     for (int i = 0; i < d.L; i++) d.fl_P[i] = mulmod(d.Mhat_mod_msk[i], d.inv_M_mod_msk, msk);
+    for (int j = 0; j < K; j++) {
+        d.mt_inv_qhat_n[j] = mulmod(d.mt_inv_qhat[j], d.tab[j].ninv, d.tab[j].mod);
+        d.fl_c_n[j] = mulmod(d.fl_c[j], d.tab[j].ninv, d.tab[j].mod);
+    }
+    for (int k = 0; k < d.S; k++) d.fl_T_n[k] = mulmod(d.fl_T[k], d.tab[K + k].ninv, d.tab[K + k].mod);
     return hp;
 }
 
diff --git a/crcnn_b200/csrc/params.h b/crcnn_b200/csrc/params.h
--- a/crcnn_b200/csrc/params.h
+++ b/crcnn_b200/csrc/params.h
@@ -53,6 +53,9 @@
     uint64_t fl_T[MAXS];
     uint64_t fl_N[MAXS][MAXK];
     uint64_t fl_P[MAXS];
+    uint64_t mt_inv_qhat_n[MAXK];
+    uint64_t fl_c_n[MAXK];
+    uint64_t fl_T_n[MAXS];
 };
 
 struct HostParams {
```

New measurement: 39.48, median of 6. 1.03x the previous value.
